# CuzImSlymi/Apertis-LLM

Measured on NVIDIA B200. Metric: SSM+MoE block fwd+bwd tokens/sec, higher is better.
Workload: dtype bf16

## Files before the change

### apertis_llm_b200/_lib.py

```python
from __future__ import annotations

import ctypes
import os
import subprocess
import threading
from ctypes import c_char_p, c_float, c_int, c_int64, c_size_t, c_uint32, c_void_p

import torch

_HERE = os.path.dirname(os.path.abspath(__file__))
LIB_PATH = os.path.join(_HERE, "libapertis_b200.so")
CSRC = os.path.join(_HERE, "csrc")

AB_F32, AB_BF16 = 0, 1
ACT = {"gelu": 0, "relu": 1, "silu": 2, "swish": 2}
EPI_NONE, EPI_BIAS, EPI_BIAS_ACT, EPI_DACT, EPI_ADD = 0, 1, 2, 3, 4
SCAN_SINGLE_PASS, SCAN_TWO_PASS, SCAN_PIPELINED, SCAN_ROUNDS = 0, 1, 2, 3
ROW_ALIGN = 256
ROUTER_EXACT, ROUTER_BF16, ROUTER_FP16 = 0, 1, 2

P, I, I64, SZ, F, U32 = c_void_p, c_int, c_int64, c_size_t, c_float, c_uint32

SIGNATURES = {
    "ab_version": (I, []),
    "ab_device_check": (I, [I]),
    "ab_last_error": (I, [c_char_p, SZ]),
    "ab_causal_conv1d_silu_fwd": (I, [P, I64, P, P, P, I, I, I, I, I, P]),
    "ab_causal_conv1d_silu_bwd_workspace_bytes": (SZ, [I, I, I]),
    "ab_causal_conv1d_silu_bwd": (I, [P, I64, P, P, P, P, I64, P, P, P, SZ, I, I, I, I, I, P]),
    "ab_selective_scan_plan": (I, [I, I, I, I, P, P, P, P, P]),
    "ab_selective_scan_fwd": (I, [P, P, P, P, I64, P, I64, P, P, P, P, P, P, P, P, SZ, U32, I, I, I, I, I, I, P]),
    "ab_selective_scan_bwd": (I, [P, P, P, P, I64, P, I64, P, P, P, P, P, P, P, P, I64, P, P, P, P, P, SZ, U32, I,
                                  I, I, I, I, I, P]),
    "ab_ssm_scan_plan": (I, [I, I, I, I, P, P]),
    "ab_ssm_scan_tune": (I, [I, I, I, I, I]),
    "ab_ssm_scan_fwd": (I, [P, I64, P, I64, P, P, P, I64, P, I64, P, P, P, P, P, P, P, P, SZ, I, I, I, I, I, P]),
    "ab_ssm_scan_bwd": (I, [P, I64, P, P, I64, P, I64, P, P, P, P, P, P, I64, P, P, I64, P, I64, P, I64, I, P, P, P, P, SZ,
                            I, I, I, I, I, P]),
    "ab_gemm_row_tile": (I, []),
    "ab_shifted_ce_fwd": (I, [P, P, P, P, P, P, I, I, I, I64, I, P]),
    "ab_shifted_ce_bwd": (I, [P, P, P, P, P, I, I, I, I64, I, P]),
    "ab_ep_permute_ln": (I, [P, P, P, P, P, P, P, P, I, I, I64, I, I, I64, I, I, P]),
    "ab_ep_unpermute_bwd": (I, [P, P, P, P, P, P, P, I, I, I64, P, F, P, I, I, I64, I, I, I, P]),
    "ab_ep_grouped_gemm_nt": (I, [P, P, P, P, P, I, I, I64, P, P, I64, I, I, I, I, I, I, P]),
    "ab_ep_grouped_gemm_nn": (I, [P, P, P, P, P, I, I, I64, P, P, I64, I, I, I, I, I, I, P]),
    "ab_moe_router_workspace_bytes": (SZ, [I, I, I]),
    "ab_moe_router_fwd": (I, [P, P, P, F, P, P, P, P, P, P, P, P, P, P, P, P, P, P, SZ, I, I, I, I, I, I, P]),
    "ab_moe_topk_from_logits": (I, [P, P, P, P, P, P, I, I, I, P]),
    "ab_moe_max_rows": (I64, [I, I, I, I, I]),
    "ab_moe_plan_workspace_bytes": (SZ, [I, I, I]),
    "ab_moe_plan": (I, [P, P, P, I, P, P, P, P, P, P, P, P, SZ, I, I, I, I, I64, I, P]),
    "ab_moe_permute_ln": (I, [P, P, P, P, P, P, P, P, I, I, I64, I, I, P]),
    "ab_moe_unpermute": (I, [P, P, P, P, P, F, P, I, I, I, I, I, P]),
    "ab_moe_unpermute_bwd": (I, [P, P, P, P, P, P, P, P, F, P, I, I, I64, I, I, I, P]),
    "ab_moe_permute_ln_bwd_workspace_bytes": (SZ, [I, I, I64]),
    "ab_moe_permute_ln_bwd": (I, [P, P, P, P, P, P, P, P, P, P, P, SZ, I, I, I, I64, I, I, P]),
    "ab_moe_segment_colsum_workspace_bytes": (SZ, [I, I, I64]),
    "ab_moe_segment_colsum": (I, [P, P, P, P, P, SZ, I, I, I, I64, I, P]),
    "ab_moe_router_bwd_workspace_bytes": (SZ, [I, I, I]),
    "ab_moe_router_bwd": (I, [P] * 24 + [SZ, I, I, I, I, I, P]),
    "ab_grouped_gemm_nt": (I, [P, P, P, P, P, P, P, P, I64, I, I, I, I, I, I, F, P, P]),
    "ab_grouped_gemm_nn": (I, [P, P, P, P, P, P, P, P, I64, I, I, I, I, I, I, F, P, P]),
    "ab_grouped_gemm_tn_workspace_bytes": (SZ, [I, I, I, I]),
    "ab_grouped_gemm_tn": (I, [P, P, P, P, I64, I, I, I, I, I64, P, SZ, P]),
    "ab_dense_gemm_nt": (I, [P, P, P, P, P, I64, I, I, I, I, P]),
    "ab_dense_gemm_nn": (I, [P, P, P, P, P, I64, I, I, I, I, P]),
    "ab_dense_gemm_tn_workspace_bytes": (SZ, [I64, I, I]),
    "ab_dense_gemm_tn": (I, [P, P, P, P, SZ, I64, I, I, P]),
    "ab_dt_compose_fwd": (I, [P, P, P, I, I, I, I, I, P]),
    "ab_dt_compose_bwd": (I, [P, P, P, P, P, I, I, I, I, P]),
    "ab_layernorm_fwd": (I, [P, P, P, F, P, P, I, I, I, I, P]),
    "ab_layernorm_bwd_workspace_bytes": (SZ, [I, I]),
    "ab_layernorm_bwd": (I, [P, P, P, P, P, P, P, P, P, SZ, I, I, I, I, P]),
    "ab_dropout_add": (I, [P, P, P, F, P, I64, I, I, P]),
    "ab_cast_f32_to_bf16": (I, [P, P, I64, P]),
    "ab_split_f32_to_bf16x3": (I, [P, P, I64, I64, I, P]),
    "ab_split_f32_to_bf16x3_rows": (I, [P, P, P, I, I64, I64, I, P]),
}

_lib = None
_lock = threading.Lock()
_checked_devices = set()


def build(verbose: bool = False) -> str:
    cmd = ["make", "-C", CSRC, "-j", "8"]
    res = subprocess.run(cmd, capture_output=True, text=True)
    if res.returncode != 0:
        raise RuntimeError("building libapertis_b200.so failed:\n" + res.stdout[-4000:] + res.stderr[-4000:])
    if verbose:
        print(res.stdout[-2000:])
    return LIB_PATH


def load() -> ctypes.CDLL:
    global _lib
    with _lock:
        if _lib is not None:
            return _lib
        if not os.path.exists(LIB_PATH):
            build()
        lib = ctypes.CDLL(LIB_PATH)
        for name, (res, args) in SIGNATURES.items():
            fn = getattr(lib, name)
            fn.restype = res
            fn.argtypes = args
        _lib = lib
        return lib


def last_error() -> str:
    buf = ctypes.create_string_buffer(600)
    load().ab_last_error(buf, 600)
    return buf.value.decode("utf-8", "replace")


def ptr(t):
    if t is None:
        return None
    return t.data_ptr()


def dt(t_or_dtype) -> int:
    d = t_or_dtype.dtype if torch.is_tensor(t_or_dtype) else t_or_dtype
    if d == torch.float32:
        return AB_F32
    if d == torch.bfloat16:
        return AB_BF16
    raise TypeError(f"apertis_b200 kernels take float32 or bfloat16 activations, got {d}")


def stream_ptr(device=None) -> int:
    return torch.cuda.current_stream(device).cuda_stream


def ensure_device(device) -> None:
    if device.type != "cuda":
        raise RuntimeError("apertis_llm_b200: the hot path only runs on a CUDA sm_100a (B200) device; got "
                           f"device '{device}'. There is no CPU fallback.")
    idx = device.index if device.index is not None else torch.cuda.current_device()
    if idx in _checked_devices:
        return
    rc = load().ab_device_check(idx)
    if rc != 0:
        raise RuntimeError("apertis_llm_b200: " + last_error())
    _checked_devices.add(idx)


KERNELS_PER_CALL = {
    "ab_causal_conv1d_silu_fwd": 1, "ab_causal_conv1d_silu_bwd": 2,
    "ab_selective_scan_fwd": 1, "ab_selective_scan_bwd": 2,
    "ab_ssm_scan_fwd": 1, "ab_ssm_scan_bwd": 2, "ab_dense_gemm_nt": 1, "ab_dense_gemm_nn": 1, "ab_dense_gemm_tn": 2,
    "ab_dt_compose_fwd": 1, "ab_dt_compose_bwd": 2,
    "ab_moe_router_fwd": 2, "ab_moe_topk_from_logits": 1, "ab_moe_plan": 2, "ab_moe_permute_ln": 1, "ab_moe_unpermute": 1,
    "ab_moe_unpermute_bwd": 1, "ab_moe_permute_ln_bwd": 2, "ab_moe_segment_colsum": 2, "ab_moe_router_bwd": 3,
    "ab_layernorm_fwd": 1, "ab_layernorm_bwd": 3,
    "ab_grouped_gemm_nt": 1, "ab_grouped_gemm_nn": 1, "ab_grouped_gemm_tn": 1, "ab_cast_f32_to_bf16": 1,
    "ab_shifted_ce_fwd": 2, "ab_shifted_ce_bwd": 1, "ab_ep_permute_ln": 1, "ab_ep_unpermute_bwd": 1, "ab_ep_grouped_gemm_nt": 1, "ab_ep_grouped_gemm_nn": 1,
    "ab_split_f32_to_bf16x3": 1, "ab_split_f32_to_bf16x3_rows": 1,
}
launch_count = 0
_timed = None


def start_timing(names):
    global _timed
    _timed = {"names": set(names), "events": []}


def stop_timing():
    global _timed
    t, _timed = _timed, None
    out = {}
    if t is None:
        return out
    torch.cuda.synchronize()
    for name, a, b in t["events"]:
        out.setdefault(name, []).append(a.elapsed_time(b))
    return out


def call(name: str, *args):
    global launch_count
    fn = getattr(load(), name)
    if _timed is not None and name in _timed["names"]:
        a, b = torch.cuda.Event(enable_timing=True), torch.cuda.Event(enable_timing=True)
        a.record()
        rc = fn(*args)
        b.record()
        _timed["events"].append((name, a, b))
    else:
        rc = fn(*args)
    if rc != 0:
        raise RuntimeError(f"{name} failed (code {rc}): {last_error()}")
    launch_count += KERNELS_PER_CALL.get(name, 1)


def query(name: str, *args):
    return getattr(load(), name)(*args)
```

### apertis_llm_b200/csrc/moe_plan.cu

```cuda
#include "common.cuh"

namespace {

template <typename T>
__device__ __forceinline__ void ld4g(const T* p, float* f) {
    if constexpr (sizeof(T) == 4) {
        const float4 q = __ldg(reinterpret_cast<const float4*>(p));
        f[0] = q.x; f[1] = q.y; f[2] = q.z; f[3] = q.w;
    } else {
        const uint2 r = __ldg(reinterpret_cast<const uint2*>(p));
        f[0] = __uint_as_float(r.x << 16); f[1] = __uint_as_float(r.x & 0xffff0000u);
        f[2] = __uint_as_float(r.y << 16); f[3] = __uint_as_float(r.y & 0xffff0000u);
    }
}

constexpr int AB_MAX_PEERS = 16;
struct PeerRows {
    unsigned char* base[AB_MAX_PEERS];
    int n, rows_per_peer, rank;
};
__device__ __forceinline__ unsigned char* peer_row(const PeerRows& pr, void* local, int64_t r, int Dm, int es) {
    if (pr.n == 0) return reinterpret_cast<unsigned char*>(local) + (size_t)r * Dm * es;
    const int d = (int)(r / pr.rows_per_peer);
    const int64_t j = r - (int64_t)d * pr.rows_per_peer;
    return pr.base[d] + ((size_t)pr.rank * pr.rows_per_peer + j) * Dm * es;
}

template <typename T>
__device__ __forceinline__ void st4(T* p, float a, float b, float c, float d) {
    if constexpr (sizeof(T) == 4) {
        *reinterpret_cast<float4*>(p) = make_float4(a, b, c, d);
    } else {
        __nv_bfloat162 lo = __floats2bfloat162_rn(a, b), hi = __floats2bfloat162_rn(c, d);
        *reinterpret_cast<uint2*>(p) = make_uint2(*reinterpret_cast<uint32_t*>(&lo), *reinterpret_cast<uint32_t*>(&hi));
    }
}

constexpr int PLAN_THREADS = 1024;

__device__ __forceinline__ int block_excl_scan(int cnt, int* warp_tot , int& total) {
    const int lane = threadIdx.x & 31, warp = threadIdx.x >> 5;
    int inc = cnt;
#pragma unroll
    for (int o = 1; o < 32; o <<= 1) {
        const int v = __shfl_up_sync(0xffffffffu, inc, o);
        if (lane >= o) inc += v;
    }
    if (lane == 31) warp_tot[warp] = inc;
    __syncthreads();
    int before = 0, tot = 0;
    const int nw = blockDim.x >> 5;
    for (int i = 0; i < nw; ++i) {
        const int c = warp_tot[i];
        if (i < warp) before += c;
        tot += c;
    }
    __syncthreads();
    total = tot;
    return before + inc - cnt;
}

constexpr int TPT = 8;

__device__ __forceinline__ void radix_select_bin(int* hist, int& need, int& sel_bin, int* s_sel_bin, int* s_need) {
    if (threadIdx.x < 32) {
        const int lane = threadIdx.x;
        int h[8], mine = 0;
#pragma unroll
        for (int i = 0; i < 8; ++i) { h[i] = hist[lane * 8 + i]; mine += h[i]; }
        int incl = mine;
#pragma unroll
        for (int o = 1; o < 32; o <<= 1) {
            const int v = __shfl_down_sync(0xffffffffu, incl, o);
            if (lane + o < 32) incl += v;
        }
        const int above = incl - mine;
        const int nd0 = need;
        const bool here = above < nd0 && above + mine >= nd0;
        const unsigned who = __ballot_sync(0xffffffffu, here);
        if (who == 0u) {
            if (lane == 0) { *s_sel_bin = 0; *s_need = nd0 - (above + mine) + h[0]; }
        } else if (lane == __ffs(who) - 1) {
            int nd = nd0 - above, bin = 7;
            for (; bin > 0; --bin) {
                if (h[bin] >= nd) break;
                nd -= h[bin];
            }
            *s_sel_bin = lane * 8 + bin;
            *s_need = nd;
        }
    }
    __syncthreads();
    sel_bin = *s_sel_bin;
    need = *s_need;
    __syncthreads();
}

__device__ __forceinline__ void hist_add_warp(int* hist, bool valid, int bin) {
    const unsigned act = __ballot_sync(0xffffffffu, valid);
    if (valid) {
        const unsigned peers = __match_any_sync(act, bin);
        if ((__ffs(peers) - 1) == (int)(threadIdx.x & 31)) atomicAdd(&hist[bin], __popc(peers));
    }
}

__global__ void __launch_bounds__(PLAN_THREADS) plan_count_kernel(const int32_t* __restrict__ idx, const float* __restrict__ w,
                                                                  const int32_t* __restrict__ active, int cap,
                                                                  int32_t* __restrict__ counts, int32_t* __restrict__ row_local,
                                                                  int S, int K, int list_cap) {
    extern __shared__ uint2 s_list[];
    __shared__ int hist[256];
    __shared__ int warp_tot[32];
    __shared__ int s_sel_bin, s_need;
    const int e = blockIdx.x;
    const int tid = threadIdx.x;
    const bool is_active = active == nullptr || active[e] != 0;
    int kept_total = 0;
    for (int k = 0; k < K; ++k) {
        int n_cand = 0;
        const int span = blockDim.x * TPT;
        for (int s0 = 0; s0 < S; s0 += span) {
            const int sb = s0 + tid * TPT;
            uint32_t wb[TPT];
            bool c[TPT];
            int mine = 0;
#pragma unroll
            for (int t = 0; t < TPT; ++t) {
                const int s = sb + t;
                c[t] = s < S && idx[(size_t)s * K + k] == e;
                wb[t] = c[t] ? __float_as_uint(w[(size_t)s * K + k]) : 0u;
                mine += c[t];
            }
            int tot;
            int pos = n_cand + block_excl_scan(mine, warp_tot, tot);
#pragma unroll
            for (int t = 0; t < TPT; ++t) {
                if (c[t]) {
                    if (pos < list_cap) s_list[pos] = make_uint2((uint32_t)(sb + t), wb[t]);
                    ++pos;
                }
            }
            n_cand += tot;
        }
        __syncthreads();
        const bool in_smem = n_cand <= list_cap;
        const int rem = cap - kept_total;
        int mode = 0;
        if (is_active && n_cand > 0 && rem > 0) mode = n_cand <= rem ? 1 : 2;
        uint32_t tau = 0;
        int n_eq_take = 0;
        if (mode == 2) {
            uint32_t prefix = 0, mask = 0;
            int need = rem, bin;
            for (int pass = 3; pass >= 0; --pass) {
                for (int i = tid; i < 256; i += blockDim.x) hist[i] = 0;
                __syncthreads();
                if (in_smem) {
                    for (int i0 = 0; i0 < n_cand; i0 += blockDim.x) {
                        const int i = i0 + tid;
                        const uint32_t b = i < n_cand ? s_list[i].y : 0u;
                        hist_add_warp(hist, i < n_cand && (b & mask) == prefix, (int)((b >> (8 * pass)) & 0xff));
                    }
                } else {
                    for (int s0 = 0; s0 < S; s0 += blockDim.x) {
                        const int s = s0 + tid;
                        const bool c = s < S && idx[(size_t)s * K + k] == e;
                        const uint32_t b = c ? __float_as_uint(w[(size_t)s * K + k]) : 0u;
                        hist_add_warp(hist, c && (b & mask) == prefix, (int)((b >> (8 * pass)) & 0xff));
                    }
                }
                __syncthreads();
                radix_select_bin(hist, need, bin, &s_sel_bin, &s_need);
                prefix |= (uint32_t)bin << (8 * pass);
                mask |= 0xffu << (8 * pass);
            }
            tau = prefix;
            n_eq_take = need;
        }
        int run_eq = 0, run_kept = 0;
        const int n_items = in_smem ? n_cand : S;
        for (int s0 = 0; s0 < n_items; s0 += span) {
            const int ib = s0 + tid * TPT;
            bool c[TPT], gt[TPT], eq[TPT];
            int tokv[TPT];
            int n_eq = 0;
#pragma unroll
            for (int t = 0; t < TPT; ++t) {
                const int i = ib + t;
                uint32_t b = 0u;
                if (in_smem) {
                    c[t] = i < n_cand;
                    if (c[t]) { const uint2 it = s_list[i]; tokv[t] = (int)it.x; b = it.y; } else tokv[t] = 0;
                } else {
                    c[t] = i < S && idx[(size_t)i * K + k] == e;
                    tokv[t] = i;
                    if (c[t]) b = __float_as_uint(w[(size_t)i * K + k]);
                }
                gt[t] = c[t] && (mode == 1 || (mode == 2 && b > tau));
                eq[t] = c[t] && mode == 2 && b == tau;
                n_eq += eq[t];
            }
            int tot_eq = 0, tot_kept = 0;
            int eq_rank = run_eq;
            if (mode == 2) eq_rank += block_excl_scan(n_eq, warp_tot, tot_eq);
            bool kept[TPT];
            int n_kept = 0;
#pragma unroll
            for (int t = 0; t < TPT; ++t) {
                kept[t] = gt[t] || (eq[t] && eq_rank < n_eq_take);
                eq_rank += eq[t];
                n_kept += kept[t];
            }
            int pos = kept_total + run_kept + block_excl_scan(n_kept, warp_tot, tot_kept);
#pragma unroll
            for (int t = 0; t < TPT; ++t) {
                if (c[t]) row_local[(size_t)tokv[t] * K + k] = kept[t] ? pos : -1;
                pos += kept[t];
            }
            run_eq += tot_eq;
            run_kept += tot_kept;
        }
        kept_total += run_kept;
        __syncthreads();
    }
    if (tid == 0) counts[e] = kept_total;
}

__global__ void plan_finalize_kernel(const int32_t* __restrict__ idx, const int32_t* __restrict__ counts,
                                     const int32_t* __restrict__ row_local, int32_t* __restrict__ seg_off,
                                     int32_t* __restrict__ row_of, int32_t* __restrict__ tok_of_row,
                                     int32_t* __restrict__ slot_of_row, int32_t* __restrict__ tile_expert,
                                     int32_t* __restrict__ n_rows, int S, int K, int E, int align, int64_t max_rows,
                                     int fixed_seg) {
    __shared__ int soff[34];
    if (threadIdx.x == 0) {
        int o = 0, kept = 0;
        for (int e = 0; e < E; ++e) {
            soff[e] = o;
            if (fixed_seg > 0 && counts[e] > fixed_seg) __trap();
            o += fixed_seg > 0 ? fixed_seg : (counts[e] + align - 1) / align * align;
            kept += counts[e];
        }
        soff[E] = o;
        soff[E + 1] = kept;
    }
    __syncthreads();
    if (blockIdx.x == 0) {
        for (int i = threadIdx.x; i <= E; i += blockDim.x) seg_off[i] = soff[i];
        if (threadIdx.x == 0) { n_rows[0] = soff[E]; n_rows[1] = soff[E + 1]; }
        const int ntiles = (int)(max_rows / align);
        for (int t = threadIdx.x; t < ntiles; t += blockDim.x) {
            const int r = t * align;
            int ex = -1;
            for (int e = 0; e < E; ++e)
                if (r >= soff[e] && r < soff[e + 1]) ex = e;
            tile_expert[t] = ex;
        }
    }
    const int64_t n = (int64_t)S * K;
    for (int64_t i = (int64_t)blockIdx.x * blockDim.x + threadIdx.x; i < n; i += (int64_t)gridDim.x * blockDim.x) {
        const int rl = row_local[i];
        if (rl >= 0) {
            const int r = soff[idx[i]] + rl;
            row_of[i] = r;
            tok_of_row[r] = (int)(i / K);
            slot_of_row[r] = (int)(i % K);
        } else {
            row_of[i] = -1;
        }
    }
}

template <typename TI, typename TO>
__global__ void __launch_bounds__(256) permute_ln_kernel(const TI* __restrict__ x, const float* __restrict__ stats,
                                                         const float* __restrict__ ln_w, const float* __restrict__ ln_b,
                                                         const int32_t* __restrict__ tok_of_row,
                                                         const int32_t* __restrict__ tile_expert,
                                                         const int32_t* __restrict__ n_rows, TO* __restrict__ xn, int Dm,
                                                         int align, const PeerRows pr) {
    const int lane = threadIdx.x & 31;
    const int wpb = blockDim.x >> 5;
    const int total = n_rows[0];
    for (int r = blockIdx.x * wpb + (threadIdx.x >> 5); r < total; r += gridDim.x * wpb) {
        const int tok = tok_of_row[r];
        TO* orow = reinterpret_cast<TO*>(peer_row(pr, xn, r, Dm, (int)sizeof(TO)));
        if (tok < 0) {
            for (int d = lane * 4; d < Dm; d += 128) st4<TO>(orow + d, 0.f, 0.f, 0.f, 0.f);
            continue;
        }
        const int e = tile_expert[r / align];
        const float mean = stats[2 * (size_t)tok], rstd = stats[2 * (size_t)tok + 1];
        const TI* irow = x + (size_t)tok * Dm;
        const float* g = ln_w + (size_t)e * Dm;
        const float* bb = ln_b + (size_t)e * Dm;
        for (int d = lane * 4; d < Dm; d += 128) {
            const float4 gv = __ldg(reinterpret_cast<const float4*>(g + d));
            const float4 bv = __ldg(reinterpret_cast<const float4*>(bb + d));
            float xv[4];
#pragma unroll
            for (int v = 0; v < 4; ++v) xv[v] = ab_to_float(irow[d + v]);
            const float o0 = fmaf((xv[0] - mean) * rstd, gv.x, bv.x), o1 = fmaf((xv[1] - mean) * rstd, gv.y, bv.y);
            const float o2 = fmaf((xv[2] - mean) * rstd, gv.z, bv.z), o3 = fmaf((xv[3] - mean) * rstd, gv.w, bv.w);
            st4<TO>(orow + d, o0, o1, o2, o3);
        }
    }
}

template <typename TY, typename TO, int KM>
__global__ void __launch_bounds__(256) unpermute_kernel(const TY* __restrict__ y, const int32_t* __restrict__ row_of,
                                                        const float* __restrict__ w, const float* __restrict__ res, TO* __restrict__ out,
                                                        const uint32_t* __restrict__ seed, uint32_t thresh, float scale, int S, int K, int Dm) {
    constexpr int DU = 8 / KM;
    const int lane = threadIdx.x & 31;
    const int wpb = blockDim.x >> 5;
    uint32_t s0 = 0, s1 = 0;
    if (seed) { s0 = __ldg(seed); s1 = __ldg(seed + 1); }
    for (int s = blockIdx.x * wpb + (threadIdx.x >> 5); s < S; s += gridDim.x * wpb) {
        TO* orow = out + (size_t)s * Dm;
        const TY* rows[KM];
        float wk[KM];
        int rid[KM];
#pragma unroll
        for (int k = 0; k < KM; ++k) {
            rid[k] = k < K ? row_of[(size_t)s * K + k] : -1;
            wk[k] = rid[k] >= 0 ? w[(size_t)s * K + k] : 0.f;
            rows[k] = rid[k] >= 0 ? y + (size_t)rid[k] * Dm : nullptr;
        }
        for (int d0 = lane * 4; d0 < Dm; d0 += 128 * DU) {
            float yv[DU][KM][4];
#pragma unroll
            for (int u = 0; u < DU; ++u) {
                const int d = d0 + u * 128;
#pragma unroll
                for (int k = 0; k < KM; ++k) {
                    if (k < K && rows[k] != nullptr && d < Dm) ld4g<TY>(rows[k] + d, yv[u][k]);
                    else { yv[u][k][0] = yv[u][k][1] = yv[u][k][2] = yv[u][k][3] = 0.f; }
                }
            }
#pragma unroll
            for (int u = 0; u < DU; ++u) {
                const int d = d0 + u * 128;
                if (d >= Dm) break;
                float acc[4] = {0.f, 0.f, 0.f, 0.f};
#pragma unroll
                for (int k = 0; k < KM; ++k) {
                    if (k < K && rows[k] != nullptr) {
#pragma unroll
                        for (int v = 0; v < 4; ++v) acc[v] += yv[u][k][v] * wk[k];
                    }
                }
                if (seed) {
#pragma unroll
                    for (int v = 0; v < 4; ++v) acc[v] = ab_out_keep(s0, s1, (uint64_t)s * Dm + d + v, thresh) ? acc[v] * scale : 0.f;
                }
                if (res) {
                    const float4 rr = *reinterpret_cast<const float4*>(res + (size_t)s * Dm + d);
                    acc[0] += rr.x; acc[1] += rr.y; acc[2] += rr.z; acc[3] += rr.w;
                }
                st4<TO>(orow + d, acc[0], acc[1], acc[2], acc[3]);
            }
        }
    }
}

template <typename TD, typename TY, typename TO>
__global__ void __launch_bounds__(256) unpermute_bwd_kernel(const TD* __restrict__ dout, const TY* __restrict__ y,
                                                            const float* __restrict__ w, const int32_t* __restrict__ tok_of_row,
                                                            const int32_t* __restrict__ slot_of_row,
                                                            const int32_t* __restrict__ n_rows, TO* __restrict__ dy,
                                                            float* __restrict__ dw_row, const uint32_t* __restrict__ seed, uint32_t thresh,
                                                            float scale, int K, int Dm, const PeerRows pr) {
    const int lane = threadIdx.x & 31;
    const int wpb = blockDim.x >> 5;
    const int total = n_rows[0];
    uint32_t s0 = 0, s1 = 0;
    if (seed) { s0 = __ldg(seed); s1 = __ldg(seed + 1); }
    for (int r = blockIdx.x * wpb + (threadIdx.x >> 5); r < total; r += gridDim.x * wpb) {
        const int tok = tok_of_row[r];
        TO* orow = reinterpret_cast<TO*>(peer_row(pr, dy, r, Dm, (int)sizeof(TO)));
        if (tok < 0) {
            for (int d = lane * 4; d < Dm; d += 128) st4<TO>(orow + d, 0.f, 0.f, 0.f, 0.f);
            if (lane == 0) dw_row[r] = 0.f;
            continue;
        }
        const float wk = w[(size_t)tok * K + slot_of_row[r]];
        const TD* drow = dout + (size_t)tok * Dm;
        const TY* yrow = y + (size_t)r * Dm;
        float dot = 0.f;
        for (int d = lane * 4; d < Dm; d += 128) {
            float o[4];
#pragma unroll
            for (int v = 0; v < 4; ++v) {
                float g = ab_to_float(drow[d + v]);
                if (seed) g = ab_out_keep(s0, s1, (uint64_t)tok * Dm + d + v, thresh) ? g * scale : 0.f;
                dot = fmaf(g, ab_to_float(yrow[d + v]), dot);
                o[v] = g * wk;
            }
            st4<TO>(orow + d, o[0], o[1], o[2], o[3]);
        }
        dot = ab_warp_sum(dot);
        if (lane == 0) dw_row[r] = dot;
    }
}

template <typename TX, typename TG>
__global__ void __launch_bounds__(256) permute_ln_bwd_rows_kernel(const TG* __restrict__ dxn, const TX* __restrict__ x,
                                                                  const float* __restrict__ stats, const float* __restrict__ ln_w,
                                                                  const int32_t* __restrict__ tok_of_row,
                                                                  const int32_t* __restrict__ tile_expert,
                                                                  const int32_t* __restrict__ n_rows, float* __restrict__ dxrow,
                                                                  int Dm, int align) {
    const int lane = threadIdx.x & 31, wpb = blockDim.x >> 5;
    const int total = n_rows[0];
    for (int r = blockIdx.x * wpb + (threadIdx.x >> 5); r < total; r += gridDim.x * wpb) {
        const int tok = tok_of_row[r];
        if (tok < 0) continue;
        const int e = tile_expert[r / align];
        const float* g = ln_w + (size_t)e * Dm;
        const float mean = stats[2 * (size_t)tok], rstd = stats[2 * (size_t)tok + 1];
        const TX* xr = x + (size_t)tok * Dm;
        const TG* gr = dxn + (size_t)r * Dm;
        float a1 = 0.f, a2 = 0.f;
        for (int d = lane * 4; d < Dm; d += 128) {
            const float4 gv = __ldg(reinterpret_cast<const float4*>(g + d));
            const float gg[4] = {gv.x, gv.y, gv.z, gv.w};
#pragma unroll
            for (int v = 0; v < 4; ++v) {
                const float dh = ab_to_float(gr[d + v]) * gg[v];
                const float xh = (ab_to_float(xr[d + v]) - mean) * rstd;
                a1 += dh;
                a2 = fmaf(dh, xh, a2);
            }
        }
        const float m1 = ab_warp_sum(a1) / (float)Dm, m2 = ab_warp_sum(a2) / (float)Dm;
        float* orow = dxrow + (size_t)r * Dm;
        for (int d = lane * 4; d < Dm; d += 128) {
            const float4 gv = __ldg(reinterpret_cast<const float4*>(g + d));
            const float gg[4] = {gv.x, gv.y, gv.z, gv.w};
            float o[4];
#pragma unroll
            for (int v = 0; v < 4; ++v) {
                const float dh = ab_to_float(gr[d + v]) * gg[v];
                const float xh = (ab_to_float(xr[d + v]) - mean) * rstd;
                o[v] = rstd * (dh - m1 - xh * m2);
            }
            *reinterpret_cast<float4*>(orow + d) = make_float4(o[0], o[1], o[2], o[3]);
        }
    }
}

template <typename TX, typename TG, int NIT>
__global__ void __launch_bounds__(256, NIT <= 6 ? 3 : 2) permute_ln_bwd_fused_kernel(const TG* __restrict__ dxn, const TX* __restrict__ x,
                                                                   const float* __restrict__ stats, const float* __restrict__ ln_w,
                                                                   const int32_t* __restrict__ tok_of_row,
                                                                   const int32_t* __restrict__ tile_expert,
                                                                   const int32_t* __restrict__ n_rows, float* __restrict__ dxrow,
                                                                   float* __restrict__ part, int Dm, int align, int ratio) {
    __shared__ float sacc[2][NIT * 128];
    const int t = blockIdx.x;
    if ((int64_t)t * align >= n_rows[0]) return;
    const int e = tile_expert[t / ratio];
    if (e < 0) return;
    const int lane = threadIdx.x & 31, warp = threadIdx.x >> 5, wpb = blockDim.x >> 5;
    const float* g = ln_w + (size_t)e * Dm;
    float gw[NIT][4], gb[NIT][4];
#pragma unroll
    for (int it = 0; it < NIT; ++it) {
#pragma unroll
        for (int v = 0; v < 4; ++v) { gw[it][v] = 0.f; gb[it][v] = 0.f; }
    }
    int tok_cur = tok_of_row[t * align + warp];
    int tok_nxt = warp + wpb < align ? tok_of_row[t * align + warp + wpb] : -1;
    for (int i = warp; i < align; i += wpb) {
        const int r = t * align + i;
        const int tok = tok_cur;
        tok_cur = tok_nxt;
        tok_nxt = i + 2 * wpb < align ? tok_of_row[t * align + i + 2 * wpb] : -1;
        if (tok_cur >= 0) {
            const char* px = reinterpret_cast<const char*>(x + (size_t)tok_cur * Dm);
            const char* pg = reinterpret_cast<const char*>(dxn + (size_t)(r + wpb) * Dm);
            for (int o = lane * 128; o < Dm * (int)sizeof(TX); o += 32 * 128) asm volatile("prefetch.global.L1 [%0];" ::"l"(px + o));
            for (int o = lane * 128; o < Dm * (int)sizeof(TG); o += 32 * 128) asm volatile("prefetch.global.L1 [%0];" ::"l"(pg + o));
        }
        if (tok < 0) continue;
        const float mean = stats[2 * (size_t)tok], rstd = stats[2 * (size_t)tok + 1];
        const TX* xr = x + (size_t)tok * Dm;
        const TG* gr = dxn + (size_t)r * Dm;
        float a1 = 0.f, a2 = 0.f;
#pragma unroll
        for (int it = 0; it < NIT; ++it) {
            const int d = it * 128 + lane * 4;
            if (d < Dm) {
                float fx[4], fg[4], gg[4];
                ld4g<TX>(xr + d, fx);
                ld4g<TG>(gr + d, fg);
                ld4g<float>(g + d, gg);
#pragma unroll
                for (int v = 0; v < 4; ++v) {
                    const float xh = (fx[v] - mean) * rstd;
                    gw[it][v] = fmaf(fg[v], xh, gw[it][v]);
                    gb[it][v] += fg[v];
                    const float dh = fg[v] * gg[v];
                    a1 += dh;
                    a2 = fmaf(dh, xh, a2);
                }
            }
        }
        const float m1 = ab_warp_sum(a1) / (float)Dm, m2 = ab_warp_sum(a2) / (float)Dm;
        float* orow = dxrow + (size_t)r * Dm;
#pragma unroll
        for (int it = 0; it < NIT; ++it) {
            const int d = it * 128 + lane * 4;
            if (d < Dm) {
                float fx[4], fg[4], gg[4], o[4];
                ld4g<TX>(xr + d, fx);
                ld4g<TG>(gr + d, fg);
                ld4g<float>(g + d, gg);
#pragma unroll
                for (int v = 0; v < 4; ++v) o[v] = rstd * (fg[v] * gg[v] - m1 - (fx[v] - mean) * rstd * m2);
                *reinterpret_cast<float4*>(orow + d) = make_float4(o[0], o[1], o[2], o[3]);
            }
        }
    }
    for (int wv = 0; wv < wpb; ++wv) {
        if (warp == wv) {
#pragma unroll
            for (int it = 0; it < NIT; ++it) {
#pragma unroll
                for (int v = 0; v < 4; ++v) {
                    const int i = it * 128 + lane * 4 + v;
                    sacc[0][i] = wv ? sacc[0][i] + gw[it][v] : gw[it][v];
                    sacc[1][i] = wv ? sacc[1][i] + gb[it][v] : gb[it][v];
                }
            }
        }
        __syncthreads();
    }
    for (int i = threadIdx.x; i < 2 * Dm; i += blockDim.x) {
        const int q = i / Dm, d = i % Dm;
        part[((size_t)t * 2 + q) * Dm + d] = sacc[q][d];
    }
}

template <typename TX, typename TG>
__global__ void __launch_bounds__(256) permute_ln_bwd_cols_kernel(const TG* __restrict__ dxn, const TX* __restrict__ x,
                                                                  const float* __restrict__ stats,
                                                                  const int32_t* __restrict__ tok_of_row,
                                                                  const int32_t* __restrict__ tile_expert,
                                                                  const int32_t* __restrict__ n_rows, float* __restrict__ part,
                                                                  int Dm, int align, int ratio) {
    __shared__ float red[8][2][128];
    const int t = blockIdx.x;
    if ((int64_t)t * align >= n_rows[0] || tile_expert[t / ratio] < 0) return;
    const int lane = threadIdx.x & 31, warp = threadIdx.x >> 5;
    const int d = blockIdx.y * 128 + lane * 4;
    float gw[4] = {0.f, 0.f, 0.f, 0.f}, gb[4] = {0.f, 0.f, 0.f, 0.f};
    if (d < Dm) {
        for (int i = warp; i < align; i += 8) {
            const int r = t * align + i;
            const int tok = tok_of_row[r];
            if (tok < 0) continue;
            const float mean = stats[2 * (size_t)tok], rstd = stats[2 * (size_t)tok + 1];
#pragma unroll
            for (int v = 0; v < 4; ++v) {
                const float dv = ab_to_float(dxn[(size_t)r * Dm + d + v]);
                const float xh = (ab_to_float(x[(size_t)tok * Dm + d + v]) - mean) * rstd;
                gw[v] = fmaf(dv, xh, gw[v]);
                gb[v] += dv;
            }
        }
    }
#pragma unroll
    for (int v = 0; v < 4; ++v) { red[warp][0][lane * 4 + v] = gw[v]; red[warp][1][lane * 4 + v] = gb[v]; }
    __syncthreads();
    const int q = threadIdx.x >> 7, c = threadIdx.x & 127;
    float s2 = 0.f;
#pragma unroll
    for (int wv = 0; wv < 8; ++wv) s2 += red[wv][q][c];
    const int dd = blockIdx.y * 128 + c;
    if (dd < Dm) part[((size_t)t * 2 + q) * Dm + dd] = s2;
}

template <typename T>
__global__ void __launch_bounds__(256) tile_colsum_kernel(const T* __restrict__ a, const int32_t* __restrict__ tile_expert,
                                                          const int32_t* __restrict__ n_rows, float* __restrict__ part, int C,
                                                          int align, int ratio) {
    __shared__ float red[8][256];
    const int t = blockIdx.x;
    if ((int64_t)t * align >= n_rows[0] || tile_expert[t / ratio] < 0) return;
    const int lane = threadIdx.x & 31, warp = threadIdx.x >> 5;
    const int c0 = blockIdx.y * 256 + lane * 8;
    float acc[8];
#pragma unroll
    for (int v = 0; v < 8; ++v) acc[v] = 0.f;
    if (c0 < C) {
        constexpr int VN = 16 / (int)sizeof(T);
        for (int i0 = warp; i0 < align; i0 += 32) {
            uint4 q[4][8 / VN];
#pragma unroll
            for (int u = 0; u < 4; ++u) {
                const int i = i0 + u * 8;
                const uint4* row = reinterpret_cast<const uint4*>(a + ((size_t)t * align + i) * C + c0);
#pragma unroll
                for (int w = 0; w < 8 / VN; ++w) q[u][w] = i < align ? __ldg(row + w) : make_uint4(0u, 0u, 0u, 0u);
            }
#pragma unroll
            for (int u = 0; u < 4; ++u) {
#pragma unroll
                for (int w = 0; w < 8 / VN; ++w) {
                    float f[VN];
                    ab_vec16<T>::unpack(q[u][w], f);
#pragma unroll
                    for (int v = 0; v < VN; ++v) acc[w * VN + v] += f[v];
                }
            }
        }
    }
#pragma unroll
    for (int v = 0; v < 8; ++v) red[warp][lane * 8 + v] = acc[v];
    __syncthreads();
    const int c = threadIdx.x;
    float s2 = 0.f;
#pragma unroll
    for (int wv = 0; wv < 8; ++wv) s2 += red[wv][c];
    if (blockIdx.y * 256 + c < C) part[(size_t)t * C + blockIdx.y * 256 + c] = s2;
}

__global__ void tile_reduce_kernel(const float* __restrict__ part, const int32_t* __restrict__ tile_expert,
                                   const int32_t* __restrict__ n_rows, float* __restrict__ out_a, float* __restrict__ out_b,
                                   int split, int ncols, int align, int ratio) {
    __shared__ int s_t0, s_t1;
    __shared__ int s_list[1024];
    __shared__ int s_n;
    const int e = blockIdx.y;
    const int ntiles = n_rows[0] / align;
    if (threadIdx.x < 32) {
        int n = 0, t0 = ntiles, t1 = 0;
        for (int base = 0; base < ntiles; base += 32) {
            const int t = base + (int)threadIdx.x;
            const bool mine = t < ntiles && tile_expert[t / ratio] == e;
            const unsigned m = __ballot_sync(0xffffffffu, mine);
            if (mine) {
                const int pos = n + __popc(m & ((1u << threadIdx.x) - 1u));
                if (pos < 1024) s_list[pos] = t;
            }
            if (m) { t0 = min(t0, base + __ffs(m) - 1); t1 = base + 32 - __clz(m); }
            n += __popc(m);
        }
        if (threadIdx.x == 0) { s_t0 = t0; s_t1 = t1; s_n = n; }
    }
    __syncthreads();
    const int j = blockIdx.x * blockDim.x + threadIdx.x;
    if (j >= ncols) return;
    float s = 0.f;
    if (s_n <= 1024) {
        for (int i0 = 0; i0 < s_n; i0 += 8) {
            float v[8];
#pragma unroll
            for (int u = 0; u < 8; ++u) v[u] = i0 + u < s_n ? part[(size_t)s_list[i0 + u] * ncols + j] : 0.f;
#pragma unroll
            for (int u = 0; u < 8; ++u) s += v[u];
        }
    } else {
        for (int t = s_t0; t < s_t1; ++t)
            if (tile_expert[t / ratio] == e) s += part[(size_t)t * ncols + j];
    }
    if (j < split) out_a[(size_t)e * split + j] = s;
    else out_b[(size_t)e * (ncols - split) + (j - split)] = s;
}

int work_rows(int row_align) { return row_align % 128 == 0 ? 128 : row_align; }

int make_peers(PeerRows* pr, const uint64_t* peer_ptrs, int W, int rank, int64_t rows_per_peer) {
    memset(pr, 0, sizeof(*pr));
    if (peer_ptrs == nullptr) return AB_OK;
    AB_REQUIRE(W >= 1 && W <= AB_MAX_PEERS && rank >= 0 && rank < W && rows_per_peer > 0 && rows_per_peer < (1ll << 31),
               "ep: bad peer table (W=%d, rank=%d, rows_per_peer=%lld; at most %d ranks)", W, rank, (long long)rows_per_peer, AB_MAX_PEERS);
    for (int i = 0; i < W; ++i) {
        AB_REQUIRE(peer_ptrs[i] != 0 && peer_ptrs[i] % 16 == 0, "ep: peer buffer %d is null or not 16-byte aligned", i);
        pr->base[i] = reinterpret_cast<unsigned char*>(peer_ptrs[i]);
    }
    pr->n = W; pr->rows_per_peer = (int)rows_per_peer; pr->rank = rank;
    return AB_OK;
}

int rows_grid(int64_t max_rows) {
    const int64_t want = ab_ceil_div(max_rows, 8);
    const int64_t cap = (int64_t)ab_num_sms() * 8;
    return (int)(want < cap ? want : cap);
}

}

extern "C" int64_t ab_moe_max_rows(int S, int K, int E, int cap, int row_align) {
    int64_t kept = (int64_t)S * K;
    if ((int64_t)E * cap < kept) kept = (int64_t)E * cap;
    return ab_round_up(kept + (int64_t)E * (row_align - 1), row_align);
}

extern "C" size_t ab_moe_plan_workspace_bytes(int S, int K, int E) {
    (void)E;
    return (size_t)ab_round_up((int64_t)S * K * sizeof(int32_t), 256);
}

extern "C" int ab_moe_plan(const int32_t* idx, const float* w, const int32_t* active, int cap, int32_t* counts,
                           int32_t* seg_off, int32_t* row_of, int32_t* tok_of_row, int32_t* slot_of_row,
                           int32_t* tile_expert, int32_t* n_rows, void* ws, size_t ws_bytes, int S, int K, int E,
                           int row_align, int64_t max_rows, int fixed_seg, cudaStream_t stream) {
    AB_REQUIRE(S > 0 && K >= 1 && E >= 1 && E <= 32, "moe_plan: bad shape S=%d K=%d E=%d", S, K, E);
    if (fixed_seg > 0) {
        AB_REQUIRE(fixed_seg % row_align == 0 && (cap >= S || fixed_seg >= cap) && max_rows == (int64_t)E * fixed_seg,
                   "moe_plan: fixed_seg (%d) must be a multiple of %d, >= cap, and max_rows == E*fixed_seg", fixed_seg, row_align);
    } else {
        AB_REQUIRE(row_align > 0 && max_rows % row_align == 0 && max_rows >= ab_moe_max_rows(S, K, E, cap < S ? cap : S, row_align),
                   "moe_plan: max_rows %lld too small or not a multiple of %d", (long long)max_rows, row_align);
    }
    AB_REQUIRE(ws && ws_bytes >= ab_moe_plan_workspace_bytes(S, K, E), "moe_plan: workspace too small");
    int32_t* row_local = (int32_t*)ws;
    AB_CHECK_CUDA(cudaMemsetAsync(tok_of_row, 0xFF, (size_t)max_rows * sizeof(int32_t), stream));
    AB_CHECK_CUDA(cudaMemsetAsync(slot_of_row, 0xFF, (size_t)max_rows * sizeof(int32_t), stream));
    int list_cap = (200 * 1024) / 8;
    if (list_cap > S) list_cap = S;
    const size_t plan_smem = (size_t)list_cap * sizeof(uint2);
    AB_CHECK_CUDA(cudaFuncSetAttribute(plan_count_kernel, cudaFuncAttributeMaxDynamicSharedMemorySize, (int)plan_smem));
    plan_count_kernel<<<E, PLAN_THREADS, plan_smem, stream>>>(idx, w, active, cap, counts, row_local, S, K, list_cap);
    AB_LAUNCH_CHECK();
    const int64_t want = ab_ceil_div((int64_t)S * K, 256);
    const int grid = (int)(want < ab_num_sms() * 4 ? want : ab_num_sms() * 4);
    plan_finalize_kernel<<<grid, 256, 0, stream>>>(idx, counts, row_local, seg_off, row_of, tok_of_row, slot_of_row, tile_expert,
                                                   n_rows, S, K, E, row_align, max_rows, fixed_seg);
    AB_LAUNCH_CHECK();
    return AB_OK;
}

namespace {
int permute_ln_impl(const void* x, const float* stats, const float* ln_w, const float* ln_b, const int32_t* tok_of_row,
                    const int32_t* tile_expert, const int32_t* n_rows, void* xn, int Dm, int row_align, int64_t max_rows, int dtype,
                    int out_dtype, const PeerRows& pr, cudaStream_t stream) {
    AB_REQUIRE(Dm > 0 && Dm % 4 == 0, "moe_permute_ln: hidden size must be a multiple of 4");
    const int grid = rows_grid(max_rows);
#define AB_PLN(TI, TO) permute_ln_kernel<TI, TO><<<grid, 256, 0, stream>>>((const TI*)x, stats, ln_w, ln_b, tok_of_row, tile_expert, n_rows, (TO*)xn, Dm, row_align, pr)
    if (dtype == AB_F32 && out_dtype == AB_F32) AB_PLN(float, float);
    else if (dtype == AB_F32 && out_dtype == AB_BF16) AB_PLN(float, __nv_bfloat16);
    else if (dtype == AB_BF16 && out_dtype == AB_BF16) AB_PLN(__nv_bfloat16, __nv_bfloat16);
    else if (dtype == AB_BF16 && out_dtype == AB_F32) AB_PLN(__nv_bfloat16, float);
    else AB_REQUIRE(false, "moe_permute_ln: bad dtypes");
#undef AB_PLN
    AB_LAUNCH_CHECK();
    return AB_OK;
}
}

extern "C" int ab_moe_permute_ln(const void* x, const float* stats, const float* ln_w, const float* ln_b,
                                 const int32_t* tok_of_row, const int32_t* tile_expert, const int32_t* n_rows, void* xn, int Dm,
                                 int row_align, int64_t max_rows, int dtype, int out_dtype, cudaStream_t stream) {
    PeerRows pr;
    make_peers(&pr, nullptr, 0, 0, 0);
    return permute_ln_impl(x, stats, ln_w, ln_b, tok_of_row, tile_expert, n_rows, xn, Dm, row_align, max_rows, dtype, out_dtype, pr, stream);
}

extern "C" int ab_ep_permute_ln(const void* x, const float* stats, const float* ln_w, const float* ln_b,
                                const int32_t* tok_of_row, const int32_t* tile_expert, const int32_t* n_rows,
                                const uint64_t* peer_xn, int W, int rank, int64_t rows_per_peer, int Dm, int row_align,
                                int64_t max_rows, int dtype, int out_dtype, cudaStream_t stream) {
    AB_REQUIRE(peer_xn != nullptr && max_rows == (int64_t)W * rows_per_peer, "ep_permute_ln: max_rows must equal W * rows_per_peer");
    PeerRows pr;
    if (int e = make_peers(&pr, peer_xn, W, rank, rows_per_peer)) return e;
    return permute_ln_impl(x, stats, ln_w, ln_b, tok_of_row, tile_expert, n_rows, nullptr, Dm, row_align, max_rows, dtype, out_dtype, pr, stream);
}

extern "C" int ab_moe_unpermute(const void* y, const int32_t* row_of, const float* w, const float* res, void* out, float drop_p,
                                const uint32_t* drop_seed, int S, int K, int Dm, int y_dtype, int out_dtype, cudaStream_t stream) {
    AB_REQUIRE(Dm > 0 && Dm % 4 == 0, "moe_unpermute: hidden size must be a multiple of 4");
    AB_REQUIRE(drop_p >= 0.f && drop_p < 1.f && (drop_p == 0.f || drop_seed), "moe_unpermute: dropout p must be in [0,1) and needs a seed when > 0");
    AB_REQUIRE(res == nullptr || ((uintptr_t)res % 16) == 0, "moe_unpermute: the residual must be 16-byte aligned fp32");
    const uint32_t thresh = (uint32_t)((double)drop_p * 4294967296.0);
    const float scale = drop_p > 0.f ? 1.0f / (1.0f - drop_p) : 1.0f;
    const uint32_t* sd = drop_p > 0.f ? drop_seed : nullptr;
    const int grid = rows_grid(S);
#define AB_UNP(TY, TO)                                                                                                          \
    {                                                                                                                            \
        if (K <= 2) unpermute_kernel<TY, TO, 2><<<grid, 256, 0, stream>>>((const TY*)y, row_of, w, res, (TO*)out, sd, thresh, scale, S, K, Dm); \
        else if (K <= 4) unpermute_kernel<TY, TO, 4><<<grid, 256, 0, stream>>>((const TY*)y, row_of, w, res, (TO*)out, sd, thresh, scale, S, K, Dm); \
        else unpermute_kernel<TY, TO, 8><<<grid, 256, 0, stream>>>((const TY*)y, row_of, w, res, (TO*)out, sd, thresh, scale, S, K, Dm); \
    }
    AB_REQUIRE(K >= 1 && K <= 8, "moe_unpermute: experts_per_token must be in [1, 8]");
    if (y_dtype == AB_F32 && out_dtype == AB_F32) AB_UNP(float, float)
    else if (y_dtype == AB_BF16 && out_dtype == AB_F32) AB_UNP(__nv_bfloat16, float)
    else if (y_dtype == AB_BF16 && out_dtype == AB_BF16) AB_UNP(__nv_bfloat16, __nv_bfloat16)
    else if (y_dtype == AB_F32 && out_dtype == AB_BF16) AB_UNP(float, __nv_bfloat16)
    else AB_REQUIRE(false, "moe_unpermute: bad dtypes");
#undef AB_UNP
    AB_LAUNCH_CHECK();
    return AB_OK;
}

namespace {
int unpermute_bwd_impl(const void* dout, const void* y, const float* w, const int32_t* tok_of_row, const int32_t* slot_of_row,
                       const int32_t* n_rows, void* dy, float* dw_row, float drop_p, const uint32_t* drop_seed, int K, int Dm,
                       int64_t max_rows, int dout_dtype, int y_dtype, int dy_dtype, const PeerRows& pr, cudaStream_t stream) {
    AB_REQUIRE(Dm > 0 && Dm % 4 == 0, "moe_unpermute_bwd: hidden size must be a multiple of 4");
    AB_REQUIRE(drop_p >= 0.f && drop_p < 1.f && (drop_p == 0.f || drop_seed), "moe_unpermute_bwd: dropout p must be in [0,1) and needs a seed when > 0");
    const uint32_t thresh = (uint32_t)((double)drop_p * 4294967296.0);
    const float scale = drop_p > 0.f ? 1.0f / (1.0f - drop_p) : 1.0f;
    const uint32_t* sd = drop_p > 0.f ? drop_seed : nullptr;
    const int grid = rows_grid(max_rows);
#define AB_UB(TD, TY, TO) unpermute_bwd_kernel<TD, TY, TO><<<grid, 256, 0, stream>>>((const TD*)dout, (const TY*)y, w, tok_of_row, slot_of_row, n_rows, (TO*)dy, dw_row, sd, thresh, scale, K, Dm, pr)
    const int key = dout_dtype * 4 + y_dtype * 2 + dy_dtype;
    switch (key) {
        case 0: AB_UB(float, float, float); break;
        case 1: AB_UB(float, float, __nv_bfloat16); break;
        case 2: AB_UB(float, __nv_bfloat16, float); break;
        case 3: AB_UB(float, __nv_bfloat16, __nv_bfloat16); break;
        case 4: AB_UB(__nv_bfloat16, float, float); break;
        case 5: AB_UB(__nv_bfloat16, float, __nv_bfloat16); break;
        case 6: AB_UB(__nv_bfloat16, __nv_bfloat16, float); break;
        case 7: AB_UB(__nv_bfloat16, __nv_bfloat16, __nv_bfloat16); break;
        default: AB_REQUIRE(false, "moe_unpermute_bwd: bad dtypes");
    }
#undef AB_UB
    AB_LAUNCH_CHECK();
    return AB_OK;
}
}

extern "C" int ab_moe_unpermute_bwd(const void* dout, const void* y, const float* w, const int32_t* tok_of_row,
                                    const int32_t* slot_of_row, const int32_t* n_rows, void* dy, float* dw_row, float drop_p,
                                    const uint32_t* drop_seed, int K, int Dm, int64_t max_rows, int dout_dtype, int y_dtype,
                                    int dy_dtype, cudaStream_t stream) {
    PeerRows pr;
    make_peers(&pr, nullptr, 0, 0, 0);
    return unpermute_bwd_impl(dout, y, w, tok_of_row, slot_of_row, n_rows, dy, dw_row, drop_p, drop_seed, K, Dm, max_rows, dout_dtype,
                              y_dtype, dy_dtype, pr, stream);
}

extern "C" int ab_ep_unpermute_bwd(const void* dout, const void* y, const float* w, const int32_t* tok_of_row,
                                   const int32_t* slot_of_row, const int32_t* n_rows, const uint64_t* peer_dy, int W, int rank,
                                   int64_t rows_per_peer, float* dw_row, float drop_p, const uint32_t* drop_seed, int K, int Dm,
                                   int64_t max_rows, int dout_dtype, int y_dtype, int dy_dtype, cudaStream_t stream) {
    AB_REQUIRE(peer_dy != nullptr && max_rows == (int64_t)W * rows_per_peer, "ep_unpermute_bwd: max_rows must equal W * rows_per_peer");
    PeerRows pr;
    if (int e = make_peers(&pr, peer_dy, W, rank, rows_per_peer)) return e;
    return unpermute_bwd_impl(dout, y, w, tok_of_row, slot_of_row, n_rows, nullptr, dw_row, drop_p, drop_seed, K, Dm, max_rows,
                              dout_dtype, y_dtype, dy_dtype, pr, stream);
}

extern "C" size_t ab_moe_permute_ln_bwd_workspace_bytes(int Dm, int row_align, int64_t max_rows) {
    return (size_t)ab_round_up((max_rows / work_rows(row_align)) * 2 * (int64_t)Dm * sizeof(float), 256);
}

extern "C" int ab_moe_permute_ln_bwd(const void* dxn, const void* x, const float* stats, const float* ln_w,
                                     const int32_t* tok_of_row, const int32_t* tile_expert, const int32_t* n_rows, float* dxrow,
                                     float* dln_w, float* dln_b, void* ws, size_t ws_bytes, int Dm, int E, int row_align,
                                     int64_t max_rows, int dtype, int dxn_dtype, cudaStream_t stream) {
    AB_REQUIRE(ws && ws_bytes >= ab_moe_permute_ln_bwd_workspace_bytes(Dm, row_align, max_rows), "moe_permute_ln_bwd: workspace too small");
    AB_REQUIRE(Dm % 4 == 0, "moe_permute_ln_bwd: hidden size must be a multiple of 4");
    const int sub = work_rows(row_align), ratio = row_align / sub;
    const int ntiles = (int)(max_rows / sub);
    float* part = (float*)ws;
    const int rgrid = rows_grid(max_rows);
    dim3 cgrid(ntiles, (unsigned)ab_ceil_div(Dm, 128));
    const int nit = (int)ab_ceil_div(Dm, 128);
#define AB_LNB_F(TX, TG, NIT)                                                                                                    \
    permute_ln_bwd_fused_kernel<TX, TG, NIT><<<ntiles, 256, 0, stream>>>((const TG*)dxn, (const TX*)x, stats, ln_w, tok_of_row, \
                                                                         tile_expert, n_rows, dxrow, part, Dm, sub, ratio)
#define AB_LNB(TX, TG)                                                                                                           \
    {                                                                                                                            \
        if (nit <= 8) {                                                                                                          \
            if (nit <= 2) AB_LNB_F(TX, TG, 2); else if (nit <= 4) AB_LNB_F(TX, TG, 4);                                           \
            else if (nit <= 6) AB_LNB_F(TX, TG, 6); else AB_LNB_F(TX, TG, 8);                                                    \
        } else {                                                                                                                 \
            permute_ln_bwd_rows_kernel<TX, TG><<<rgrid, 256, 0, stream>>>((const TG*)dxn, (const TX*)x, stats, ln_w, tok_of_row, \
                                                                          tile_expert, n_rows, dxrow, Dm, row_align);            \
            permute_ln_bwd_cols_kernel<TX, TG><<<cgrid, 256, 0, stream>>>((const TG*)dxn, (const TX*)x, stats, tok_of_row,       \
                                                                          tile_expert, n_rows, part, Dm, sub, ratio);            \
        }                                                                                                                        \
    }
    if (dtype == AB_F32 && dxn_dtype == AB_F32) AB_LNB(float, float)
    else if (dtype == AB_F32 && dxn_dtype == AB_BF16) AB_LNB(float, __nv_bfloat16)
    else if (dtype == AB_BF16 && dxn_dtype == AB_BF16) AB_LNB(__nv_bfloat16, __nv_bfloat16)
    else if (dtype == AB_BF16 && dxn_dtype == AB_F32) AB_LNB(__nv_bfloat16, float)
    else AB_REQUIRE(false, "moe_permute_ln_bwd: bad dtypes");
#undef AB_LNB
#undef AB_LNB_F
    AB_LAUNCH_CHECK();
    dim3 grid((unsigned)ab_ceil_div(2 * Dm, 128), E);
    tile_reduce_kernel<<<grid, 128, 0, stream>>>(part, tile_expert, n_rows, dln_w, dln_b, Dm, 2 * Dm, sub, ratio);
    AB_LAUNCH_CHECK();
    return AB_OK;
}

extern "C" size_t ab_moe_segment_colsum_workspace_bytes(int C, int row_align, int64_t max_rows) {
    return (size_t)ab_round_up((max_rows / work_rows(row_align)) * (int64_t)C * sizeof(float), 256);
}

extern "C" int ab_moe_segment_colsum(const void* a, const int32_t* tile_expert, const int32_t* n_rows, float* out, void* ws,
                                     size_t ws_bytes, int C, int E, int row_align, int64_t max_rows, int dtype,
                                     cudaStream_t stream) {
    AB_REQUIRE(ws && ws_bytes >= ab_moe_segment_colsum_workspace_bytes(C, row_align, max_rows), "moe_segment_colsum: workspace too small");
    const int sub = work_rows(row_align), ratio = row_align / sub;
    const int ntiles = (int)(max_rows / sub);
    float* part = (float*)ws;
    AB_REQUIRE(C % 8 == 0 && ((uintptr_t)a % 16) == 0, "moe_segment_colsum: column count must be a multiple of 8 and the matrix 16-byte aligned");
    dim3 cgrid(ntiles, (unsigned)ab_ceil_div(C, 256));
    if (dtype == AB_F32) tile_colsum_kernel<float><<<cgrid, 256, 0, stream>>>((const float*)a, tile_expert, n_rows, part, C, sub, ratio);
    else tile_colsum_kernel<__nv_bfloat16><<<cgrid, 256, 0, stream>>>((const __nv_bfloat16*)a, tile_expert, n_rows, part, C, sub, ratio);
    AB_LAUNCH_CHECK();
    dim3 grid((unsigned)ab_ceil_div(C, 128), E);
    tile_reduce_kernel<<<grid, 128, 0, stream>>>(part, tile_expert, n_rows, out, nullptr, C, C, sub, ratio);
    AB_LAUNCH_CHECK();
    return AB_OK;
}
```

### apertis_llm_b200/csrc/moe_router.cu

```cuda
#include <cuda_fp16.h>

#include "common.cuh"

namespace {

constexpr int WARPS = 8;
constexpr int MAX_K = 8;

__device__ __forceinline__ float ab_round_to(float v, int quant) {
    if (quant == AB_ROUTER_BF16) return __bfloat162float(__float2bfloat16_rn(v));
    if (quant == AB_ROUTER_FP16) return __half2float(__float2half_rn(v));
    return v;
}

template <typename T>
__device__ __forceinline__ void row_load(const T* row, int i, float* f) {
    ab_vec16<T>::unpack(__ldg(reinterpret_cast<const uint4*>(row) + i), f);
}

__device__ __forceinline__ void select_topk(float logit, int lane, int E, int K, float& g, float& lse, int& my_idx, float& my_p,
                                            float& den, unsigned& sel_mask) {
    const float lv = lane < E ? logit : -INFINITY;
    const float m = ab_warp_max(lv);
    const float ex = lane < E ? expf(lv - m) : 0.f;
    const float sum = ab_warp_sum(ex);
    g = ex / sum;
    lse = m + logf(sum);
    float cand = lane < E ? g : -INFINITY;
    my_idx = 0; my_p = 0.f; den = 0.f; sel_mask = 0u;
    for (int k = 0; k < K; ++k) {
        const float best = ab_warp_max(cand);
        const unsigned ball = __ballot_sync(0xffffffffu, cand == best);
        const int win = __ffs(ball) - 1;
        if (lane == k) { my_idx = win; my_p = best; }
        den += best;
        sel_mask |= 1u << win;
        if (lane == win) cand = -INFINITY;
    }
    den += 1e-6f;
}

__device__ __forceinline__ void write_selection(int s, int lane, int E, int K, float g, float lse, int my_idx, float my_p, float den,
                                                float* gates, int32_t* idx, float* probs, float* w, float* lse_out) {
    if (lane < E) gates[(size_t)s * E + lane] = g;
    if (lane < K) {
        idx[(size_t)s * K + lane] = my_idx;
        probs[(size_t)s * K + lane] = my_p;
        w[(size_t)s * K + lane] = my_p / den;
    }
    if (lane == 0) lse_out[s] = lse;
}

template <typename T, int EM>
__global__ void __launch_bounds__(WARPS * 32) router_fwd_kernel(const T* __restrict__ x, const float* __restrict__ ln_w,
                                                                const float* __restrict__ ln_b, float eps,
                                                                const float* __restrict__ Wr, const float* __restrict__ br,
                                                                const float* __restrict__ noise,
                                                                const float* __restrict__ noise_scale, float* __restrict__ lclean,
                                                                float* __restrict__ logits, float* __restrict__ gates,
                                                                int32_t* __restrict__ idx, float* __restrict__ probs,
                                                                float* __restrict__ w, float* __restrict__ lse_out,
                                                                float* __restrict__ stats, float* __restrict__ part, int S,
                                                                int Dm, int E, int K, int quant) {
    constexpr int V = ab_vec16<T>::N;
    extern __shared__ float sm[];
    float* G = sm;
    float* cvec = G + (size_t)E * Dm;
    float* red = cvec + 32;
    float* lnw_s = red + WARPS * (2 * E + 1);
    float* lnb_s = lnw_s + Dm;
    const int tid = threadIdx.x, lane = tid & 31, warp = tid >> 5;
    if (quant == AB_ROUTER_EXACT) {
        for (int e = 0; e < E; ++e)
            for (int d = tid; d < Dm; d += blockDim.x) G[(size_t)e * Dm + d] = ln_w[d] * Wr[(size_t)e * Dm + d];
        for (int e = warp; e < E; e += WARPS) {
            float acc = 0.f;
            for (int d = lane; d < Dm; d += 32) acc = fmaf(ln_b[d], Wr[(size_t)e * Dm + d], acc);
            acc = ab_warp_sum(acc);
            if (lane == 0) cvec[e] = acc + br[e];
        }
    } else {
        for (int e = 0; e < E; ++e)
            for (int d = tid; d < Dm; d += blockDim.x) G[(size_t)e * Dm + d] = ab_round_to(Wr[(size_t)e * Dm + d], quant);
        for (int d = tid; d < Dm; d += blockDim.x) { lnw_s[d] = ln_w[d]; lnb_s[d] = ln_b[d]; }
        if (tid < E) cvec[tid] = ab_round_to(br[tid], quant);
    }
    __syncthreads();
    const int nvec = Dm / V;
    float a_g = 0.f, a_cnt = 0.f, a_l2 = 0.f;
    for (int s = blockIdx.x * WARPS + warp; s < S; s += gridDim.x * WARPS) {
        const T* row = x + (size_t)s * Dm;
        float sum = 0.f;
        for (int i = lane; i < nvec; i += 32) {
            float f[V];
            row_load<T>(row, i, f);
#pragma unroll
            for (int v = 0; v < V; ++v) sum += f[v];
        }
        const float mean = ab_warp_sum(sum) / (float)Dm;
        float var = 0.f;
        float dot[EM];
#pragma unroll
        for (int e = 0; e < EM; ++e) dot[e] = 0.f;
        for (int i = lane; i < nvec; i += 32) {
            float f[V];
            row_load<T>(row, i, f);
#pragma unroll
            for (int v = 0; v < V; ++v) { f[v] -= mean; var = fmaf(f[v], f[v], var); }
#pragma unroll
            for (int e = 0; e < EM; ++e) {
                if (e < E) {
#pragma unroll
                    for (int v4 = 0; v4 < V; v4 += 4) {
                        const float4 gq = *reinterpret_cast<const float4*>(G + (size_t)e * Dm + i * V + v4);
                        dot[e] = fmaf(f[v4], gq.x, dot[e]); dot[e] = fmaf(f[v4 + 1], gq.y, dot[e]);
                        dot[e] = fmaf(f[v4 + 2], gq.z, dot[e]); dot[e] = fmaf(f[v4 + 3], gq.w, dot[e]);
                    }
                }
            }
        }
        var = ab_warp_sum(var) / (float)Dm;
        const float rstd = rsqrtf(var + eps);
        if (quant != AB_ROUTER_EXACT) {
#pragma unroll
            for (int e = 0; e < EM; ++e) dot[e] = 0.f;
            for (int i = lane; i < nvec; i += 32) {
                float f[V];
                row_load<T>(row, i, f);
#pragma unroll
                for (int v = 0; v < V; ++v) f[v] = ab_round_to(fmaf((f[v] - mean) * rstd, lnw_s[i * V + v], lnb_s[i * V + v]), quant);
#pragma unroll
                for (int e = 0; e < EM; ++e) {
                    if (e < E) {
#pragma unroll
                        for (int v = 0; v < V; ++v) dot[e] = fmaf(f[v], G[(size_t)e * Dm + i * V + v], dot[e]);
                    }
                }
            }
        }
        float mylogit = 0.f;
#pragma unroll
        for (int e = 0; e < EM; ++e) {
            if (e < E) {
                const float t = ab_warp_sum(dot[e]);
                if (lane == e) mylogit = t;
            }
        }
        float lc = 0.f;
        if (lane < E) {
            lc = quant == AB_ROUTER_EXACT ? fmaf(rstd, mylogit, cvec[lane]) : ab_round_to(mylogit + cvec[lane], quant);
            mylogit = lc;
            if (noise) mylogit = fmaf(noise[(size_t)s * E + lane], noise_scale[lane], lc);
            if (lclean) lclean[(size_t)s * E + lane] = lc;
            if (logits) logits[(size_t)s * E + lane] = mylogit;
        }
        if (lane == 0) { stats[2 * (size_t)s] = mean; stats[2 * (size_t)s + 1] = rstd; }
        float g, lse, my_p, den;
        int my_idx;
        unsigned sel_mask;
        select_topk(mylogit, lane, E, K, g, lse, my_idx, my_p, den, sel_mask);
        write_selection(s, lane, E, K, g, lse, my_idx, my_p, den, gates, idx, probs, w, lse_out);
        if (lane < E) {
            a_g += g;
            a_cnt += (sel_mask >> lane) & 1u ? 1.f : 0.f;
        }
        if (lane == 0) a_l2 = fmaf(lse, lse, a_l2);
    }
    const int NA = 2 * E + 1;
    if (lane < E) { red[warp * NA + lane] = a_g; red[warp * NA + E + lane] = a_cnt; }
    if (lane == 0) red[warp * NA + 2 * E] = a_l2;
    __syncthreads();
    if (tid < NA) {
        float s2 = 0.f;
        for (int wv = 0; wv < WARPS; ++wv) s2 += red[wv * NA + tid];
        part[(size_t)blockIdx.x * NA + tid] = s2;
    }
}

template <int EM>
__device__ __forceinline__ float reduce_dots_to_lane(float (&dot)[EM], int lane, int E) {
    float mine = 0.f;
    if (EM == 8) {
        float v4[4], v2[2], v1;
        const bool h16 = lane & 16, h8 = lane & 8, h4 = lane & 4;
#pragma unroll
        for (int j = 0; j < 4; ++j) {
            const float keep = h16 ? dot[4 + j] : dot[j], send = h16 ? dot[j] : dot[4 + j];
            v4[j] = keep + __shfl_xor_sync(0xffffffffu, send, 16);
        }
#pragma unroll
        for (int j = 0; j < 2; ++j) {
            const float keep = h8 ? v4[2 + j] : v4[j], send = h8 ? v4[j] : v4[2 + j];
            v2[j] = keep + __shfl_xor_sync(0xffffffffu, send, 8);
        }
        {
            const float keep = h4 ? v2[1] : v2[0], send = h4 ? v2[0] : v2[1];
            v1 = keep + __shfl_xor_sync(0xffffffffu, send, 4);
        }
        v1 += __shfl_xor_sync(0xffffffffu, v1, 2);
        v1 += __shfl_xor_sync(0xffffffffu, v1, 1);
        const int src = ((lane >> 2) & 1) << 4 | ((lane >> 1) & 1) << 3 | (lane & 1) << 2;
        mine = __shfl_sync(0xffffffffu, v1, src);
        if (lane >= E) mine = 0.f;
    } else {
#pragma unroll
        for (int e = 0; e < EM; ++e) {
            if (e < E) {
                const float t = ab_warp_sum(dot[e]);
                if (lane == e) mine = t;
            }
        }
    }
    return mine;
}

template <typename T, int EM, int NV>
__global__ void __launch_bounds__(WARPS * 32, (NV * ab_vec16<T>::N <= 24 && EM <= 8) ? 4 : 1) router_fwd_reg_kernel(const T* __restrict__ x, const float* __restrict__ ln_w,
                                                                    const float* __restrict__ ln_b, float eps,
                                                                    const float* __restrict__ Wr, const float* __restrict__ br,
                                                                    const float* __restrict__ noise,
                                                                    const float* __restrict__ noise_scale, float* __restrict__ lclean,
                                                                    float* __restrict__ logits, float* __restrict__ gates,
                                                                    int32_t* __restrict__ idx, float* __restrict__ probs,
                                                                    float* __restrict__ w, float* __restrict__ lse_out,
                                                                    float* __restrict__ stats, float* __restrict__ part, int S,
                                                                    int Dm, int E, int K, int quant) {
    constexpr int V = ab_vec16<T>::N;
    extern __shared__ float sm[];
    float* G = sm;
    float* cvec = G + (size_t)E * Dm;
    float* red = cvec + 32;
    float* lnw_s = red + WARPS * (2 * E + 1);
    float* lnb_s = lnw_s + Dm;
    const int tid = threadIdx.x, lane = tid & 31, warp = tid >> 5;
    if (quant == AB_ROUTER_EXACT) {
        for (int i = tid; i < E * Dm; i += blockDim.x) G[i] = ln_w[i % Dm] * Wr[i];
        for (int e = warp; e < E; e += WARPS) {
            float acc = 0.f;
            for (int d = lane; d < Dm; d += 32) acc = fmaf(ln_b[d], Wr[(size_t)e * Dm + d], acc);
            acc = ab_warp_sum(acc);
            if (lane == 0) cvec[e] = acc + br[e];
        }
    } else {
        for (int i = tid; i < E * Dm; i += blockDim.x) G[i] = ab_round_to(Wr[i], quant);
        for (int d = tid; d < Dm; d += blockDim.x) { lnw_s[d] = ln_w[d]; lnb_s[d] = ln_b[d]; }
        if (tid < E) cvec[tid] = ab_round_to(br[tid], quant);
    }
    __syncthreads();
    const int nvec = Dm / V;
    const float inv_dm = 1.0f / (float)Dm;
    float a_g = 0.f, a_cnt = 0.f, a_l2 = 0.f;
    for (int s = blockIdx.x * WARPS + warp; s < S; s += gridDim.x * WARPS) {
        const T* row = x + (size_t)s * Dm;
        float f[NV][V];
        float sum = 0.f;
#pragma unroll
        for (int i = 0; i < NV; ++i) {
            const int iv = i * 32 + lane;
            if (iv < nvec) {
                row_load<T>(row, iv, f[i]);
#pragma unroll
                for (int v = 0; v < V; ++v) sum += f[i][v];
            } else {
#pragma unroll
                for (int v = 0; v < V; ++v) f[i][v] = 0.f;
            }
        }
        const float mean = ab_warp_sum(sum) * inv_dm;
        float var = 0.f;
#pragma unroll
        for (int i = 0; i < NV; ++i) {
            if (i * 32 + lane < nvec) {
#pragma unroll
                for (int v = 0; v < V; ++v) { f[i][v] -= mean; var = fmaf(f[i][v], f[i][v], var); }
            }
        }
        var = ab_warp_sum(var) * inv_dm;
        const float rstd = rsqrtf(var + eps);
        float dot[EM];
#pragma unroll
        for (int e = 0; e < EM; ++e) dot[e] = 0.f;
#pragma unroll
        for (int i = 0; i < NV; ++i) {
            const int iv = i * 32 + lane;
            if (iv < nvec) {
                if (quant != AB_ROUTER_EXACT) {
#pragma unroll
                    for (int v4 = 0; v4 < V; v4 += 4) {
                        const float4 lw = *reinterpret_cast<const float4*>(lnw_s + iv * V + v4);
                        const float4 lb = *reinterpret_cast<const float4*>(lnb_s + iv * V + v4);
                        f[i][v4] = ab_round_to(fmaf(f[i][v4] * rstd, lw.x, lb.x), quant);
                        f[i][v4 + 1] = ab_round_to(fmaf(f[i][v4 + 1] * rstd, lw.y, lb.y), quant);
                        f[i][v4 + 2] = ab_round_to(fmaf(f[i][v4 + 2] * rstd, lw.z, lb.z), quant);
                        f[i][v4 + 3] = ab_round_to(fmaf(f[i][v4 + 3] * rstd, lw.w, lb.w), quant);
                    }
                }
#pragma unroll
                for (int e = 0; e < EM; ++e) {
                    if (e < E) {
#pragma unroll
                        for (int v4 = 0; v4 < V; v4 += 4) {
                            const float4 gq = *reinterpret_cast<const float4*>(G + (size_t)e * Dm + iv * V + v4);
                            dot[e] = fmaf(f[i][v4], gq.x, dot[e]); dot[e] = fmaf(f[i][v4 + 1], gq.y, dot[e]);
                            dot[e] = fmaf(f[i][v4 + 2], gq.z, dot[e]); dot[e] = fmaf(f[i][v4 + 3], gq.w, dot[e]);
                        }
                    }
                }
            }
        }
        float mylogit = reduce_dots_to_lane<EM>(dot, lane, E);
        float lc = 0.f;
        if (lane < E) {
            lc = quant == AB_ROUTER_EXACT ? fmaf(rstd, mylogit, cvec[lane]) : ab_round_to(mylogit + cvec[lane], quant);
            mylogit = lc;
            if (noise) mylogit = fmaf(noise[(size_t)s * E + lane], noise_scale[lane], lc);
            if (lclean) lclean[(size_t)s * E + lane] = lc;
            if (logits) logits[(size_t)s * E + lane] = mylogit;
        }
        if (lane == 0) { stats[2 * (size_t)s] = mean; stats[2 * (size_t)s + 1] = rstd; }
        float g, lse, my_p, den;
        int my_idx;
        unsigned sel_mask;
        select_topk(mylogit, lane, E, K, g, lse, my_idx, my_p, den, sel_mask);
        write_selection(s, lane, E, K, g, lse, my_idx, my_p, den, gates, idx, probs, w, lse_out);
        if (lane < E) {
            a_g += g;
            a_cnt += (sel_mask >> lane) & 1u ? 1.f : 0.f;
        }
        if (lane == 0) a_l2 = fmaf(lse, lse, a_l2);
    }
    const int NA = 2 * E + 1;
    if (lane < E) { red[warp * NA + lane] = a_g; red[warp * NA + E + lane] = a_cnt; }
    if (lane == 0) red[warp * NA + 2 * E] = a_l2;
    __syncthreads();
    if (tid < NA) {
        float s2 = 0.f;
        for (int wv = 0; wv < WARPS; ++wv) s2 += red[wv * NA + tid];
        part[(size_t)blockIdx.x * NA + tid] = s2;
    }
}

__global__ void reduce_rows_kernel(const float* __restrict__ part, int nrows, int ncols, float* __restrict__ out) {
    const int c = blockIdx.x * (blockDim.x >> 5) + (threadIdx.x >> 5);
    const int lane = threadIdx.x & 31;
    if (c >= ncols) return;
    float s = 0.f;
    for (int r = lane; r < nrows; r += 32) s += part[(size_t)r * ncols + c];
    s = ab_warp_sum(s);
    if (lane == 0) out[c] = s;
}

__global__ void __launch_bounds__(WARPS * 32) topk_from_logits_kernel(const float* __restrict__ logits, float* __restrict__ gates,
                                                                      int32_t* __restrict__ idx, float* __restrict__ probs,
                                                                      float* __restrict__ w, float* __restrict__ lse_out, int S,
                                                                      int E, int K) {
    const int lane = threadIdx.x & 31, warp = threadIdx.x >> 5;
    for (int s = blockIdx.x * WARPS + warp; s < S; s += gridDim.x * WARPS) {
        const float l = lane < E ? logits[(size_t)s * E + lane] : 0.f;
        float g, lse, my_p, den;
        int my_idx;
        unsigned sel_mask;
        select_topk(l, lane, E, K, g, lse, my_idx, my_p, den, sel_mask);
        write_selection(s, lane, E, K, g, lse, my_idx, my_p, den, gates, idx, probs, w, lse_out);
    }
}

template <typename T, int EM>
__global__ void __launch_bounds__(WARPS * 32) router_bwd_kernel(const T* __restrict__ x, const float* __restrict__ stats,
                                                                const float* __restrict__ ln_w, const float* __restrict__ ln_b,
                                                                const float* __restrict__ Wr, const float* __restrict__ br,
                                                                const float* __restrict__ gates, const int32_t* __restrict__ idx,
                                                                const float* __restrict__ probs, const float* __restrict__ lse,
                                                                const float* __restrict__ lclean, const float* __restrict__ noise,
                                                                const float* __restrict__ f, const float* __restrict__ scal,
                                                                const float* __restrict__ dw_row, const float* __restrict__ dxrow,
                                                                const int32_t* __restrict__ row_of, T* __restrict__ dx,
                                                                float* __restrict__ dlogits, float* __restrict__ part, int S,
                                                                int Dm, int E, int K) {
    constexpr int V = ab_vec16<T>::N;
    extern __shared__ float sm[];
    float* Wsm = sm;
    float* gam = Wsm + (size_t)E * Dm;
    float* GS = gam + Dm;
    float* cvec = GS + 32;
    float* red = cvec + 32;
    const int tid = threadIdx.x, lane = tid & 31, warp = tid >> 5;
    for (int i = tid; i < E * Dm; i += blockDim.x) Wsm[i] = Wr[i];
    for (int i = tid; i < Dm; i += blockDim.x) gam[i] = ln_w[i];
    for (int e = warp; e < E; e += WARPS) {
        float a1 = 0.f, a2 = 0.f;
        for (int d = lane; d < Dm; d += 32) {
            a1 = fmaf(ln_w[d], Wr[(size_t)e * Dm + d], a1);
            a2 = fmaf(ln_b[d], Wr[(size_t)e * Dm + d], a2);
        }
        a1 = ab_warp_sum(a1); a2 = ab_warp_sum(a2);
        if (lane == 0) { GS[e] = a1; cvec[e] = a2 + br[e]; }
    }
    __syncthreads();
    const float g_lb = scal[0], g_rz = scal[1];
    const int nvec = Dm / V;
    float a_db = 0.f, a_dn = 0.f;
    for (int s = blockIdx.x * WARPS + warp; s < S; s += gridDim.x * WARPS) {
        int my_r = -1, my_i = 0;
        float my_dw = 0.f, my_pk = 0.f;
        if (lane < K) {
            my_r = row_of[(size_t)s * K + lane];
            my_i = idx[(size_t)s * K + lane];
            my_pk = probs[(size_t)s * K + lane];
            my_dw = my_r >= 0 ? dw_row[my_r] : 0.f;
        }
        float den = 0.f;
        for (int k = 0; k < K; ++k) den += __shfl_sync(0xffffffffu, my_pk, k);
        den += 1e-6f;
        const float dot = ab_warp_sum(my_dw * my_pk);
        const float inv = 1.f / den;
        const float my_dp = my_dw * inv - dot * inv * inv;
        float dgate = 0.f, g = 0.f;
        for (int k = 0; k < K; ++k) {
            const int ik = __shfl_sync(0xffffffffu, my_i, k);
            const float dpk = __shfl_sync(0xffffffffu, my_dp, k);
            if (lane == ik) dgate += dpk;
        }
        if (lane < E) {
            g = gates[(size_t)s * E + lane];
            dgate = fmaf(g_lb, f[lane], dgate);
        } else {
            dgate = 0.f;
        }
        const float gd = ab_warp_sum(g * dgate);
        float dl = 0.f;
        if (lane < E) {
            dl = g * (dgate - gd) + g_rz * 2.f * lse[s] * g;
            dlogits[(size_t)s * E + lane] = dl;
            a_db += dl;
            if (noise) a_dn = fmaf(dl, noise[(size_t)s * E + lane], a_dn);
        }
        const float mean = stats[2 * (size_t)s], rstd = stats[2 * (size_t)s + 1];
        float t1 = 0.f, t2 = 0.f;
        if (lane < E) {
            t1 = dl * GS[lane];
            t2 = dl * (lclean[(size_t)s * E + lane] - cvec[lane]);
        }
        const float m1 = ab_warp_sum(t1) / (float)Dm;
        const float m2 = ab_warp_sum(t2) / (float)Dm;
        float dle[EM];
#pragma unroll
        for (int e = 0; e < EM; ++e) dle[e] = __shfl_sync(0xffffffffu, dl, e);
        int rk[MAX_K];
#pragma unroll
        for (int k = 0; k < MAX_K; ++k) { const int r = __shfl_sync(0xffffffffu, my_r, k); rk[k] = k < K ? r : -1; }
        const T* row = x + (size_t)s * Dm;
        T* orow = dx + (size_t)s * Dm;
        for (int i = lane; i < nvec; i += 32) {
            float fx[V], o[V];
            row_load<T>(row, i, fx);
            float dxn[V];
#pragma unroll
            for (int v = 0; v < V; ++v) dxn[v] = 0.f;
#pragma unroll
            for (int e = 0; e < EM; ++e) {
                if (e < E) {
#pragma unroll
                    for (int v4 = 0; v4 < V; v4 += 4) {
                        const float4 wq = *reinterpret_cast<const float4*>(Wsm + (size_t)e * Dm + i * V + v4);
                        dxn[v4] = fmaf(dle[e], wq.x, dxn[v4]); dxn[v4 + 1] = fmaf(dle[e], wq.y, dxn[v4 + 1]);
                        dxn[v4 + 2] = fmaf(dle[e], wq.z, dxn[v4 + 2]); dxn[v4 + 3] = fmaf(dle[e], wq.w, dxn[v4 + 3]);
                    }
                }
            }
#pragma unroll
            for (int v4 = 0; v4 < V; v4 += 4) {
                const float4 gq = *reinterpret_cast<const float4*>(gam + i * V + v4);
                const float gg[4] = {gq.x, gq.y, gq.z, gq.w};
#pragma unroll
                for (int u = 0; u < 4; ++u) {
                    const float xh = (fx[v4 + u] - mean) * rstd;
                    o[v4 + u] = rstd * (dxn[v4 + u] * gg[u] - m1 - xh * m2);
                }
            }
#pragma unroll
            for (int k = 0; k < MAX_K; ++k) {
                const int rkk = rk[k];
                if (rkk >= 0) {
                    const float* er = dxrow + (size_t)rkk * Dm + i * V;
#pragma unroll
                    for (int v4 = 0; v4 < V; v4 += 4) {
                        const float4 q = __ldg(reinterpret_cast<const float4*>(er + v4));
                        o[v4] += q.x; o[v4 + 1] += q.y; o[v4 + 2] += q.z; o[v4 + 3] += q.w;
                    }
                }
            }
            *(reinterpret_cast<uint4*>(orow) + i) = ab_vec16<T>::pack(o);
        }
    }
    const int NA = 2 * E;
    if (lane < E) { red[warp * NA + lane] = a_db; red[warp * NA + E + lane] = a_dn; }
    __syncthreads();
    if (tid < NA) {
        float s2 = 0.f;
        for (int wv = 0; wv < WARPS; ++wv) s2 += red[wv * NA + tid];
        part[(size_t)blockIdx.x * NA + tid] = s2;
    }
}

constexpr int qb_for(int em) { return 2048 / em; }
int em_for(int E) { return E <= 8 ? 8 : (E <= 16 ? 16 : 32); }
template <typename T, int EM>
__global__ void __launch_bounds__(256) router_q_kernel(const T* __restrict__ x, const float* __restrict__ stats,
                                                       const float* __restrict__ dlogits, float* __restrict__ qpart, int S,
                                                       int Dm, int E) {
    constexpr int QB = qb_for(EM);
    __shared__ float sdl[QB * EM];
    __shared__ float sst[QB * 2];
    const int s0 = blockIdx.y * QB;
    const int ns = min(QB, S - s0);
    for (int i = threadIdx.x; i < ns * E; i += blockDim.x) sdl[i] = dlogits[(size_t)s0 * E + i];
    for (int i = threadIdx.x; i < ns * 2; i += blockDim.x) sst[i] = stats[(size_t)s0 * 2 + i];
    __syncthreads();
    const int d = blockIdx.x * blockDim.x + threadIdx.x;
    if (d >= Dm) return;
    float acc[EM];
#pragma unroll
    for (int e = 0; e < EM; ++e) acc[e] = 0.f;
    for (int j0 = 0; j0 < ns; j0 += 8) {
        float xv[8];
#pragma unroll
        for (int u = 0; u < 8; ++u) xv[u] = j0 + u < ns ? ab_to_float(x[(size_t)(s0 + j0 + u) * Dm + d]) : 0.f;
#pragma unroll
        for (int u = 0; u < 8; ++u) {
            const int j = j0 + u;
            if (j < ns) {
                const float xh = (xv[u] - sst[2 * j]) * sst[2 * j + 1];
#pragma unroll
                for (int e = 0; e < EM; ++e)
                    if (e < E) acc[e] = fmaf(sdl[j * E + e], xh, acc[e]);
            }
        }
    }
#pragma unroll
    for (int e = 0; e < EM; ++e)
        if (e < E) qpart[((size_t)blockIdx.y * E + e) * Dm + d] = acc[e];
}

__global__ void router_param_kernel(const float* __restrict__ qpart, int nqb, const float* __restrict__ part, int nparts,
                                    const float* __restrict__ ln_w, const float* __restrict__ ln_b, const float* __restrict__ Wr,
                                    float* __restrict__ dWr, float* __restrict__ dbr, float* __restrict__ dln_w,
                                    float* __restrict__ dln_b, float* __restrict__ dnoise_scale, int Dm, int E) {
    __shared__ float sdb[64];
    __shared__ float sgw[32][33], sgb[32][33];
    __shared__ float spart[16][64];
    const int tx = threadIdx.x, e = threadIdx.y;
    const int tid = e * 32 + tx;
    const int nthr = 32 * E;
    {
        const int ncol = 2 * E;
        const int ngrp = min(16, nthr / ncol);
        const int col = tid % ncol, grp = tid / ncol;
        if (grp < ngrp) {
            float s = 0.f;
            for (int r0 = grp; r0 < nparts; r0 += ngrp * 4) {
                float v[4];
#pragma unroll
                for (int u = 0; u < 4; ++u) v[u] = r0 + u * ngrp < nparts ? part[(size_t)(r0 + u * ngrp) * ncol + col] : 0.f;
#pragma unroll
                for (int u = 0; u < 4; ++u) s += v[u];
            }
            spart[grp][col] = s;
        }
        __syncthreads();
        if (tid < ncol) {
            float s = 0.f;
            for (int g2 = 0; g2 < ngrp; ++g2) s += spart[g2][tid];
            sdb[tid] = s;
            if (blockIdx.x == 0) {
                if (tid < E) dbr[tid] = s;
                else if (dnoise_scale) dnoise_scale[tid - E] = s;
            }
        }
    }
    __syncthreads();
    const int d = blockIdx.x * 32 + tx;
    float gw = 0.f, gb = 0.f;
    if (d < Dm) {
        float q = 0.f;
        for (int r0 = 0; r0 < nqb; r0 += 8) {
            float qv[8];
#pragma unroll
            for (int u = 0; u < 8; ++u) qv[u] = r0 + u < nqb ? qpart[((size_t)(r0 + u) * E + e) * Dm + d] : 0.f;
#pragma unroll
            for (int u = 0; u < 8; ++u) q += qv[u];
        }
        const float wv = Wr[(size_t)e * Dm + d];
        dWr[(size_t)e * Dm + d] = fmaf(ln_w[d], q, ln_b[d] * sdb[e]);
        gw = wv * q;
        gb = wv * sdb[e];
    }
    sgw[e][tx] = gw;
    sgb[e][tx] = gb;
    __syncthreads();
    if (e == 0 && d < Dm) {
        float a = 0.f, b = 0.f;
        for (int i = 0; i < E; ++i) { a += sgw[i][tx]; b += sgb[i][tx]; }
        dln_w[d] = a;
        dln_b[d] = b;
    }
}

int router_grid(int S) {
    const int want = (int)ab_ceil_div(S, WARPS);
    const int cap = ab_num_sms() * 4;
    return want < cap ? want : cap;
}

struct FwdWs { size_t part_off, total; int grid; };
FwdWs fwd_ws(int S, int E) {
    FwdWs w;
    w.grid = router_grid(S);
    w.part_off = 0;
    w.total = ab_round_up((int64_t)w.grid * (2 * E + 1) * sizeof(float), 256);
    return w;
}
struct BwdWs { size_t part_off, dl_off, q_off, total; int grid, nqb; };
BwdWs bwd_ws(int S, int Dm, int E) {
    BwdWs w;
    w.grid = router_grid(S);
    w.nqb = (int)ab_ceil_div(S, qb_for(em_for(E)));
    size_t o = 0;
    w.part_off = o; o += ab_round_up((int64_t)w.grid * 2 * E * sizeof(float), 256);
    w.dl_off = o; o += ab_round_up((int64_t)S * E * sizeof(float), 256);
    w.q_off = o; o += ab_round_up((int64_t)w.nqb * E * Dm * sizeof(float), 256);
    w.total = o;
    return w;
}

int check_router(int S, int Dm, int E, int K, int dtype) {
    AB_REQUIRE(S > 0 && Dm > 0, "moe_router: empty shape S=%d Dm=%d", S, Dm);
    AB_REQUIRE(E >= 1 && E <= 32, "moe_router: num_experts must be in [1,32] (got %d)", E);
    AB_REQUIRE(K >= 1 && K <= MAX_K && K <= E, "moe_router: experts_per_token must be in [1,%d] and <= E (got %d)", MAX_K, K);
    AB_REQUIRE(dtype == AB_F32 || dtype == AB_BF16, "moe_router: bad dtype %d", dtype);
    const int V = dtype == AB_F32 ? 4 : 8;
    AB_REQUIRE(Dm % V == 0, "moe_router: hidden size %d must be a multiple of %d", Dm, V);
    return AB_OK;
}

}

extern "C" size_t ab_moe_router_workspace_bytes(int S, int Dm, int E) { (void)Dm; return fwd_ws(S, E).total; }

extern "C" int ab_moe_router_fwd(const void* x, const float* ln_w, const float* ln_b, float eps, const float* Wr,
                                 const float* br, const float* noise, const float* noise_scale, float* lclean, float* logits,
                                 float* gates, int32_t* idx, float* probs, float* w, float* lse, float* stats_out, float* aux,
                                 void* ws, size_t ws_bytes, int S, int Dm, int E, int K, int dtype, int quant, cudaStream_t stream) {
    if (int e = check_router(S, Dm, E, K, dtype)) return e;
    const FwdWs wl = fwd_ws(S, E);
    AB_REQUIRE(ws && ws_bytes >= wl.total, "moe_router_fwd: workspace too small");
    AB_REQUIRE(noise == nullptr || noise_scale != nullptr, "moe_router_fwd: noise without noise_scale");
    AB_REQUIRE(quant == AB_ROUTER_EXACT || quant == AB_ROUTER_BF16 || quant == AB_ROUTER_FP16, "moe_router_fwd: bad logit rounding mode %d", quant);
    const size_t smem = ((size_t)E * Dm + 32 + WARPS * (2 * E + 1) + 2 * (size_t)Dm) * sizeof(float);
    float* part = (float*)ws;
    const int V = dtype == AB_F32 ? 4 : 8;
    const int nv = (int)ab_ceil_div(Dm, 32 * V);
#define AB_ROUTER_LAUNCH(KERNEL)                                                                                        \
    {                                                                                                                    \
        auto k = KERNEL;                                                                                                 \
        AB_CHECK_CUDA(cudaFuncSetAttribute(k, cudaFuncAttributeMaxDynamicSharedMemorySize, (int)smem));                 \
        k<<<wl.grid, WARPS * 32, smem, stream>>>((const TT*)x, ln_w, ln_b, eps, Wr, br, noise, noise_scale, lclean,     \
                                                 logits, gates, idx, probs, w, lse, stats_out, part, S, Dm, E, K, quant); \
    }
#define AB_ROUTER_FWD(TT_, EMV)                                                                                         \
    {                                                                                                                    \
        using TT = TT_;                                                                                                  \
        if (nv <= 4) AB_ROUTER_LAUNCH((router_fwd_reg_kernel<TT, EMV, 4>))                                               \
        else if (nv <= 6) AB_ROUTER_LAUNCH((router_fwd_reg_kernel<TT, EMV, 6>))                                          \
        else if (nv <= 8) AB_ROUTER_LAUNCH((router_fwd_reg_kernel<TT, EMV, 8>))                                          \
        else if (nv <= 16 && EMV <= 8) AB_ROUTER_LAUNCH((router_fwd_reg_kernel<TT, EMV, 16>))                            \
        else AB_ROUTER_LAUNCH((router_fwd_kernel<TT, EMV>))                                                              \
    }
    if (dtype == AB_F32) {
        if (E <= 8) AB_ROUTER_FWD(float, 8) else if (E <= 16) AB_ROUTER_FWD(float, 16) else AB_ROUTER_FWD(float, 32)
    } else {
        if (E <= 8) AB_ROUTER_FWD(__nv_bfloat16, 8) else if (E <= 16) AB_ROUTER_FWD(__nv_bfloat16, 16) else AB_ROUTER_FWD(__nv_bfloat16, 32)
    }
#undef AB_ROUTER_LAUNCH
#undef AB_ROUTER_FWD
    AB_LAUNCH_CHECK();
    reduce_rows_kernel<<<(unsigned)ab_ceil_div(2 * E + 1, 4), 128, 0, stream>>>(part, wl.grid, 2 * E + 1, aux);
    AB_LAUNCH_CHECK();
    return AB_OK;
}

extern "C" int ab_moe_topk_from_logits(const float* logits, float* gates, int32_t* idx, float* probs, float* w, float* lse,
                                       int S, int E, int K, cudaStream_t stream) {
    if (int e = check_router(S, 8, E, K, AB_F32)) return e;
    topk_from_logits_kernel<<<router_grid(S), WARPS * 32, 0, stream>>>(logits, gates, idx, probs, w, lse, S, E, K);
    AB_LAUNCH_CHECK();
    return AB_OK;
}

extern "C" size_t ab_moe_router_bwd_workspace_bytes(int S, int Dm, int E) { return bwd_ws(S, Dm, E).total; }

extern "C" int ab_moe_router_bwd(const void* x, const float* stats, const float* ln_w, const float* ln_b, const float* Wr,
                                 const float* br, const float* gates, const int32_t* idx, const float* probs, const float* lse,
                                 const float* lclean, const float* noise, const float* f, const float* scal,
                                 const float* dw_row, const float* dxrow, const int32_t* row_of, void* dx, float* dWr,
                                 float* dbr, float* dln_w, float* dln_b, float* dnoise_scale, void* ws, size_t ws_bytes, int S,
                                 int Dm, int E, int K, int dtype, cudaStream_t stream) {
    if (int e = check_router(S, Dm, E, K, dtype)) return e;
    AB_REQUIRE(Dm % 4 == 0, "moe_router_bwd: hidden size must be a multiple of 4");
    const BwdWs wl = bwd_ws(S, Dm, E);
    AB_REQUIRE(ws && ws_bytes >= wl.total, "moe_router_bwd: workspace too small");
    unsigned char* w8 = (unsigned char*)ws;
    float* part = (float*)(w8 + wl.part_off);
    float* dl = (float*)(w8 + wl.dl_off);
    float* qpart = (float*)(w8 + wl.q_off);
    const size_t smem = ((size_t)E * Dm + Dm + 64 + WARPS * 2 * E) * sizeof(float);
    dim3 qgrid((unsigned)ab_ceil_div(Dm, 256), wl.nqb);
#define AB_ROUTER_BWD(TT, EMV)                                                                                          \
    {                                                                                                                    \
        auto k = router_bwd_kernel<TT, EMV>;                                                                             \
        AB_CHECK_CUDA(cudaFuncSetAttribute(k, cudaFuncAttributeMaxDynamicSharedMemorySize, (int)smem));                 \
        k<<<wl.grid, WARPS * 32, smem, stream>>>((const TT*)x, stats, ln_w, ln_b, Wr, br, gates, idx, probs, lse,       \
                                                 lclean, noise, f, scal, dw_row, dxrow, row_of, (TT*)dx, dl, part, S,   \
                                                 Dm, E, K);                                                              \
        AB_LAUNCH_CHECK();                                                                                               \
        router_q_kernel<TT, EMV><<<qgrid, 256, 0, stream>>>((const TT*)x, stats, dl, qpart, S, Dm, E);                  \
    }
    if (dtype == AB_F32) {
        if (E <= 8) AB_ROUTER_BWD(float, 8) else if (E <= 16) AB_ROUTER_BWD(float, 16) else AB_ROUTER_BWD(float, 32)
    } else {
        if (E <= 8) AB_ROUTER_BWD(__nv_bfloat16, 8) else if (E <= 16) AB_ROUTER_BWD(__nv_bfloat16, 16) else AB_ROUTER_BWD(__nv_bfloat16, 32)
    }
#undef AB_ROUTER_BWD
    AB_LAUNCH_CHECK();
    router_param_kernel<<<(unsigned)ab_ceil_div(Dm, 32), dim3(32, E), 0, stream>>>(qpart, wl.nqb, part, wl.grid, ln_w, ln_b, Wr, dWr,
                                                                                  dbr, dln_w, dln_b, dnoise_scale, Dm, E);
    AB_LAUNCH_CHECK();
    return AB_OK;
}
```

Before: 14.56 million.

## Parallelize MoE plan across token chunks and fuse router bwd kernels

The MoE capacity planning moves from one 1024-thread block per expert to a multi-CTA pipeline. It runs a grid-wide histogram radix select with last-CTA finalization, then per-chunk counts and a position kernel that uses warp match and ballot. The router forward becomes persistent with a grid capped by occupancy, and the router backward gains a fused token kernel plus a column kernel when E and Dm allow. The param kernel also gets a third grid dimension of groups. This trades a few serial launches for more small kernels and global atomics, which adds launch overhead and extra complexity.

Result: faster. 15.03 million (median of 6 runs) (+3.2%).

```diff
diff --git a/apertis_llm_b200/_lib.py b/apertis_llm_b200/_lib.py
--- a/apertis_llm_b200/_lib.py
+++ b/apertis_llm_b200/_lib.py
@@ -152,7 +152,7 @@
     "ab_selective_scan_fwd": 1, "ab_selective_scan_bwd": 2,
     "ab_ssm_scan_fwd": 1, "ab_ssm_scan_bwd": 2, "ab_dense_gemm_nt": 1, "ab_dense_gemm_nn": 1, "ab_dense_gemm_tn": 2,
     "ab_dt_compose_fwd": 1, "ab_dt_compose_bwd": 2,
-    "ab_moe_router_fwd": 2, "ab_moe_topk_from_logits": 1, "ab_moe_plan": 2, "ab_moe_permute_ln": 1, "ab_moe_unpermute": 1,
+    "ab_moe_router_fwd": 2, "ab_moe_topk_from_logits": 1, "ab_moe_plan": 7, "ab_moe_permute_ln": 1, "ab_moe_unpermute": 1,
     "ab_moe_unpermute_bwd": 1, "ab_moe_permute_ln_bwd": 2, "ab_moe_segment_colsum": 2, "ab_moe_router_bwd": 3,
     "ab_layernorm_fwd": 1, "ab_layernorm_bwd": 3,
     "ab_grouped_gemm_nt": 1, "ab_grouped_gemm_nn": 1, "ab_grouped_gemm_tn": 1, "ab_cast_f32_to_bf16": 1,
diff --git a/apertis_llm_b200/csrc/moe_plan.cu b/apertis_llm_b200/csrc/moe_plan.cu
--- a/apertis_llm_b200/csrc/moe_plan.cu
+++ b/apertis_llm_b200/csrc/moe_plan.cu
@@ -36,64 +36,47 @@
     }
 }
 
-constexpr int PLAN_THREADS = 1024;
-
-__device__ __forceinline__ int block_excl_scan(int cnt, int* warp_tot , int& total) {
-    const int lane = threadIdx.x & 31, warp = threadIdx.x >> 5;
-    int inc = cnt;
+constexpr int PLAN_THREADS = 256;
+constexpr int PLAN_CHUNK = PLAN_THREADS;
+constexpr int HIST_TOKENS = PLAN_THREADS;
+
+struct PlanSel {
+    uint32_t prefix;
+    int need;
+    int mode;
+    int base;
+};
+
+__device__ __forceinline__ void warp_select_bin(const int* hist, int lane, int& need, int& sel_bin) {
+    int h[8], mine = 0;
+#pragma unroll
+    for (int i = 0; i < 8; ++i) { h[i] = hist[lane * 8 + i]; mine += h[i]; }
+    int incl = mine;
 #pragma unroll
     for (int o = 1; o < 32; o <<= 1) {
-        const int v = __shfl_up_sync(0xffffffffu, inc, o);
-        if (lane >= o) inc += v;
-    }
-    if (lane == 31) warp_tot[warp] = inc;
-    __syncthreads();
-    int before = 0, tot = 0;
-    const int nw = blockDim.x >> 5;
-    for (int i = 0; i < nw; ++i) {
-        const int c = warp_tot[i];
-        if (i < warp) before += c;
-        tot += c;
-    }
-    __syncthreads();
-    total = tot;
-    return before + inc - cnt;
-}
-
-constexpr int TPT = 8;
-
-__device__ __forceinline__ void radix_select_bin(int* hist, int& need, int& sel_bin, int* s_sel_bin, int* s_need) {
-    if (threadIdx.x < 32) {
-        const int lane = threadIdx.x;
-        int h[8], mine = 0;
-#pragma unroll
-        for (int i = 0; i < 8; ++i) { h[i] = hist[lane * 8 + i]; mine += h[i]; }
-        int incl = mine;
-#pragma unroll
-        for (int o = 1; o < 32; o <<= 1) {
-            const int v = __shfl_down_sync(0xffffffffu, incl, o);
-            if (lane + o < 32) incl += v;
-        }
-        const int above = incl - mine;
-        const int nd0 = need;
-        const bool here = above < nd0 && above + mine >= nd0;
-        const unsigned who = __ballot_sync(0xffffffffu, here);
-        if (who == 0u) {
-            if (lane == 0) { *s_sel_bin = 0; *s_need = nd0 - (above + mine) + h[0]; }
-        } else if (lane == __ffs(who) - 1) {
-            int nd = nd0 - above, bin = 7;
-            for (; bin > 0; --bin) {
-                if (h[bin] >= nd) break;
-                nd -= h[bin];
-            }
-            *s_sel_bin = lane * 8 + bin;
-            *s_need = nd;
-        }
-    }
-    __syncthreads();
-    sel_bin = *s_sel_bin;
-    need = *s_need;
-    __syncthreads();
+        const int v = __shfl_down_sync(0xffffffffu, incl, o);
+        if (lane + o < 32) incl += v;
+    }
+    const int above = incl - mine;
+    const int nd0 = need;
+    const bool here = above < nd0 && above + mine >= nd0;
+    const unsigned who = __ballot_sync(0xffffffffu, here);
+    int bin = 0, nd = 0;
+    if (who == 0u) {
+        nd = __shfl_sync(0xffffffffu, nd0 - (above + mine) + h[0], 0);
+        bin = 0;
+    } else {
+        const int src = __ffs(who) - 1;
+        int b = 7, n2 = nd0 - above;
+        for (; b > 0; --b) {
+            if (h[b] >= n2) break;
+            n2 -= h[b];
+        }
+        bin = __shfl_sync(0xffffffffu, lane * 8 + b, src);
+        nd = __shfl_sync(0xffffffffu, n2, src);
+    }
+    sel_bin = bin;
+    need = nd;
 }
 
 __device__ __forceinline__ void hist_add_warp(int* hist, bool valid, int bin) {
@@ -104,126 +87,168 @@
     }
 }
 
-__global__ void __launch_bounds__(PLAN_THREADS) plan_count_kernel(const int32_t* __restrict__ idx, const float* __restrict__ w,
-                                                                  const int32_t* __restrict__ active, int cap,
-                                                                  int32_t* __restrict__ counts, int32_t* __restrict__ row_local,
-                                                                  int S, int K, int list_cap) {
-    extern __shared__ uint2 s_list[];
-    __shared__ int hist[256];
-    __shared__ int warp_tot[32];
-    __shared__ int s_sel_bin, s_need;
-    const int e = blockIdx.x;
-    const int tid = threadIdx.x;
-    const bool is_active = active == nullptr || active[e] != 0;
-    int kept_total = 0;
-    for (int k = 0; k < K; ++k) {
-        int n_cand = 0;
-        const int span = blockDim.x * TPT;
-        for (int s0 = 0; s0 < S; s0 += span) {
-            const int sb = s0 + tid * TPT;
-            uint32_t wb[TPT];
-            bool c[TPT];
-            int mine = 0;
-#pragma unroll
-            for (int t = 0; t < TPT; ++t) {
-                const int s = sb + t;
-                c[t] = s < S && idx[(size_t)s * K + k] == e;
-                wb[t] = c[t] ? __float_as_uint(w[(size_t)s * K + k]) : 0u;
-                mine += c[t];
-            }
-            int tot;
-            int pos = n_cand + block_excl_scan(mine, warp_tot, tot);
-#pragma unroll
-            for (int t = 0; t < TPT; ++t) {
-                if (c[t]) {
-                    if (pos < list_cap) s_list[pos] = make_uint2((uint32_t)(sb + t), wb[t]);
-                    ++pos;
-                }
-            }
-            n_cand += tot;
-        }
+__device__ __forceinline__ bool last_cta(int* ticket) {
+    __shared__ bool s_last;
+    __threadfence();
+    __syncthreads();
+    if (threadIdx.x == 0) s_last = atomicAdd(ticket, 1) == (int)(gridDim.x * gridDim.y) - 1;
+    __syncthreads();
+    if (s_last) __threadfence();
+    return s_last;
+}
+
+__global__ void __launch_bounds__(PLAN_THREADS) plan_hist_kernel(const int32_t* __restrict__ idx, const float* __restrict__ w,
+                                                                 const int32_t* __restrict__ active, int cap, int pass,
+                                                                 int* __restrict__ ghist, PlanSel* __restrict__ sel,
+                                                                 int* __restrict__ any_select, int* __restrict__ ticket,
+                                                                 int32_t* __restrict__ counts, int S, int K, int E) {
+    __shared__ int hist[32 * 256];
+    if (pass < 3 && *any_select == 0) return;
+    const int k = blockIdx.y, tid = threadIdx.x;
+    for (int i = tid; i < E * 256; i += blockDim.x) hist[i] = 0;
+    __syncthreads();
+    const int shift = 8 * pass;
+    const uint32_t mask = pass == 3 ? 0u : 0xffffffffu << (shift + 8);
+    const int s_end = min(S, (int)(blockIdx.x + 1) * HIST_TOKENS);
+    for (int s0 = blockIdx.x * HIST_TOKENS; s0 < s_end; s0 += blockDim.x) {
+        const int s = s0 + tid;
+        bool c = s < s_end;
+        int e = 0;
+        uint32_t b = 0u;
+        if (c) {
+            e = idx[(size_t)s * K + k];
+            b = __float_as_uint(w[(size_t)s * K + k]);
+            if (pass < 3) {
+                const PlanSel st = sel[e * K + k];
+                c = st.mode == 2 && (b & mask) == st.prefix;
+            }
+        }
+        hist_add_warp(hist, c, e * 256 + (int)((b >> shift) & 0xffu));
+    }
+    __syncthreads();
+    int* gh = ghist + (size_t)k * 256;
+    for (int i = tid; i < E * 256; i += blockDim.x) {
+        const int h = hist[i];
+        if (h) atomicAdd(&gh[(size_t)(i >> 8) * K * 256 + (i & 255)], h);
+    }
+    if (!last_cta(ticket)) return;
+    const int lane = tid & 31, warp = tid >> 5;
+    int any = 0;
+    for (int e = warp; e < E; e += blockDim.x >> 5) {
+        int kept = 0;
+        for (int kk = 0; kk < K; ++kk) {
+            const int* hk = ghist + ((size_t)e * K + kk) * 256;
+            PlanSel st;
+            if (pass == 3) {
+                int n = 0;
+                for (int i = lane; i < 256; i += 32) n += hk[i];
+                n = __reduce_add_sync(0xffffffffu, n);
+                const bool is_active = active == nullptr || active[e] != 0;
+                const int rem = cap - kept;
+                st.mode = 0;
+                if (is_active && n > 0 && rem > 0) st.mode = n <= rem ? 1 : 2;
+                st.base = kept;
+                st.need = rem;
+                st.prefix = 0u;
+                kept += st.mode == 1 ? n : (st.mode == 2 ? rem : 0);
+            } else {
+                st = sel[e * K + kk];
+            }
+            if (st.mode == 2) {
+                int bin;
+                warp_select_bin(hk, lane, st.need, bin);
+                st.prefix |= (uint32_t)bin << shift;
+                any = 1;
+            }
+            if (lane == 0) sel[e * K + kk] = st;
+        }
+        if (pass == 3 && lane == 0) counts[e] = kept;
+    }
+    if (pass == 3) {
+        __shared__ int s_any;
+        if (tid == 0) s_any = 0;
         __syncthreads();
-        const bool in_smem = n_cand <= list_cap;
-        const int rem = cap - kept_total;
-        int mode = 0;
-        if (is_active && n_cand > 0 && rem > 0) mode = n_cand <= rem ? 1 : 2;
-        uint32_t tau = 0;
-        int n_eq_take = 0;
-        if (mode == 2) {
-            uint32_t prefix = 0, mask = 0;
-            int need = rem, bin;
-            for (int pass = 3; pass >= 0; --pass) {
-                for (int i = tid; i < 256; i += blockDim.x) hist[i] = 0;
-                __syncthreads();
-                if (in_smem) {
-                    for (int i0 = 0; i0 < n_cand; i0 += blockDim.x) {
-                        const int i = i0 + tid;
-                        const uint32_t b = i < n_cand ? s_list[i].y : 0u;
-                        hist_add_warp(hist, i < n_cand && (b & mask) == prefix, (int)((b >> (8 * pass)) & 0xff));
-                    }
-                } else {
-                    for (int s0 = 0; s0 < S; s0 += blockDim.x) {
-                        const int s = s0 + tid;
-                        const bool c = s < S && idx[(size_t)s * K + k] == e;
-                        const uint32_t b = c ? __float_as_uint(w[(size_t)s * K + k]) : 0u;
-                        hist_add_warp(hist, c && (b & mask) == prefix, (int)((b >> (8 * pass)) & 0xff));
-                    }
-                }
-                __syncthreads();
-                radix_select_bin(hist, need, bin, &s_sel_bin, &s_need);
-                prefix |= (uint32_t)bin << (8 * pass);
-                mask |= 0xffu << (8 * pass);
-            }
-            tau = prefix;
-            n_eq_take = need;
-        }
-        int run_eq = 0, run_kept = 0;
-        const int n_items = in_smem ? n_cand : S;
-        for (int s0 = 0; s0 < n_items; s0 += span) {
-            const int ib = s0 + tid * TPT;
-            bool c[TPT], gt[TPT], eq[TPT];
-            int tokv[TPT];
-            int n_eq = 0;
-#pragma unroll
-            for (int t = 0; t < TPT; ++t) {
-                const int i = ib + t;
-                uint32_t b = 0u;
-                if (in_smem) {
-                    c[t] = i < n_cand;
-                    if (c[t]) { const uint2 it = s_list[i]; tokv[t] = (int)it.x; b = it.y; } else tokv[t] = 0;
-                } else {
-                    c[t] = i < S && idx[(size_t)i * K + k] == e;
-                    tokv[t] = i;
-                    if (c[t]) b = __float_as_uint(w[(size_t)i * K + k]);
-                }
-                gt[t] = c[t] && (mode == 1 || (mode == 2 && b > tau));
-                eq[t] = c[t] && mode == 2 && b == tau;
-                n_eq += eq[t];
-            }
-            int tot_eq = 0, tot_kept = 0;
-            int eq_rank = run_eq;
-            if (mode == 2) eq_rank += block_excl_scan(n_eq, warp_tot, tot_eq);
-            bool kept[TPT];
-            int n_kept = 0;
-#pragma unroll
-            for (int t = 0; t < TPT; ++t) {
-                kept[t] = gt[t] || (eq[t] && eq_rank < n_eq_take);
-                eq_rank += eq[t];
-                n_kept += kept[t];
-            }
-            int pos = kept_total + run_kept + block_excl_scan(n_kept, warp_tot, tot_kept);
-#pragma unroll
-            for (int t = 0; t < TPT; ++t) {
-                if (c[t]) row_local[(size_t)tokv[t] * K + k] = kept[t] ? pos : -1;
-                pos += kept[t];
-            }
-            run_eq += tot_eq;
-            run_kept += tot_kept;
-        }
-        kept_total += run_kept;
+        if (any && lane == 0) s_any = 1;
         __syncthreads();
-    }
-    if (tid == 0) counts[e] = kept_total;
+        if (tid == 0) *any_select = s_any;
+    }
+}
+
+__device__ __forceinline__ int plan_class(const PlanSel& st, uint32_t b) {
+    if (st.mode == 1) return 0;
+    if (st.mode == 2) return b > st.prefix ? 0 : (b == st.prefix ? 1 : -1);
+    return -1;
+}
+
+__global__ void __launch_bounds__(PLAN_THREADS) plan_chunk_count_kernel(const int32_t* __restrict__ idx, const float* __restrict__ w,
+                                                                        const PlanSel* __restrict__ sel, int* __restrict__ cc,
+                                                                        int S, int K, int E) {
+    __shared__ int cnt[64];
+    const int k = blockIdx.y, tid = threadIdx.x;
+    if (tid < 2 * E) cnt[tid] = 0;
+    __syncthreads();
+    const int s = blockIdx.x * PLAN_CHUNK + tid;
+    int cls = -1, e = 0;
+    if (s < S) {
+        e = idx[(size_t)s * K + k];
+        cls = plan_class(sel[e * K + k], __float_as_uint(w[(size_t)s * K + k]));
+    }
+    hist_add_warp(cnt, cls >= 0, e * 2 + (cls > 0 ? 1 : 0));
+    __syncthreads();
+    if (tid < 2 * E) cc[((size_t)blockIdx.x * K + k) * 2 * E + tid] = cnt[tid];
+}
+
+__global__ void __launch_bounds__(PLAN_THREADS) plan_pos_kernel(const int32_t* __restrict__ idx, const float* __restrict__ w,
+                                                                const PlanSel* __restrict__ sel, const int* __restrict__ cc,
+                                                                int32_t* __restrict__ row_local, int S, int K, int E) {
+    __shared__ int wcnt[PLAN_THREADS / 32][64];
+    __shared__ int sbase[PLAN_THREADS];
+    const int k = blockIdx.y, tid = threadIdx.x, lane = tid & 31, warp = tid >> 5;
+    {
+        const int ncol = 2 * E, ng = PLAN_THREADS / ncol, col = tid % ncol, grp = tid / ncol;
+        int sum = 0;
+        if (grp < ng)
+            for (int c = grp; c < (int)blockIdx.x; c += ng) sum += cc[((size_t)c * K + k) * ncol + col];
+        sbase[tid] = sum;
+    }
+    const int s = blockIdx.x * PLAN_CHUNK + tid;
+    int cls = -1, e = 0;
+    PlanSel st{0u, 0, 0, 0};
+    if (s < S) {
+        e = idx[(size_t)s * K + k];
+        st = sel[e * K + k];
+        cls = plan_class(st, __float_as_uint(w[(size_t)s * K + k]));
+    }
+    const unsigned valid = __ballot_sync(0xffffffffu, s < S);
+    const unsigned same = __match_any_sync(0xffffffffu, s < S ? e : -1) & valid;
+    const unsigned gtm = __ballot_sync(0xffffffffu, cls == 0), eqm = __ballot_sync(0xffffffffu, cls == 1);
+    const unsigned lt = (1u << lane) - 1u;
+    for (int i = tid; i < (PLAN_THREADS / 32) * 64; i += blockDim.x) (&wcnt[0][0])[i] = 0;
+    __syncthreads();
+    if (s < S && (__ffs(same) - 1) == lane) {
+        wcnt[warp][2 * e] = __popc(same & gtm);
+        wcnt[warp][2 * e + 1] = __popc(same & eqm);
+    }
+    __syncthreads();
+    if (tid < 2 * E) {
+        int run = 0;
+        for (int g = 0; g < PLAN_THREADS / (2 * E); ++g) run += sbase[g * 2 * E + tid];
+        for (int wv = 0; wv < PLAN_THREADS / 32; ++wv) {
+            const int v = wcnt[wv][tid];
+            wcnt[wv][tid] = run;
+            run += v;
+        }
+    }
+    __syncthreads();
+    if (s < S) {
+        int r = -1;
+        if (cls >= 0) {
+            const int gt_before = wcnt[warp][2 * e] + __popc(same & gtm & lt);
+            const int eq_before = wcnt[warp][2 * e + 1] + __popc(same & eqm & lt);
+            if (cls == 0 || eq_before < st.need) r = st.base + gt_before + min(eq_before, st.need);
+        }
+        row_local[(size_t)s * K + k] = r;
+    }
 }
 
 __global__ void plan_finalize_kernel(const int32_t* __restrict__ idx, const int32_t* __restrict__ counts,
@@ -698,10 +723,22 @@
     return ab_round_up(kept + (int64_t)E * (row_align - 1), row_align);
 }
 
-extern "C" size_t ab_moe_plan_workspace_bytes(int S, int K, int E) {
-    (void)E;
-    return (size_t)ab_round_up((int64_t)S * K * sizeof(int32_t), 256);
-}
+namespace {
+struct PlanWs { size_t hist_off, zero_bytes, sel_off, cc_off, total; };
+PlanWs plan_ws(int S, int K, int E) {
+    PlanWs p;
+    size_t o = ab_round_up((int64_t)S * K * sizeof(int32_t), 256);
+    p.hist_off = o;
+    p.zero_bytes = ab_round_up(((int64_t)4 * E * K * 256 + 16) * sizeof(int), 256);
+    o += p.zero_bytes;
+    p.sel_off = o; o += ab_round_up((int64_t)E * K * sizeof(PlanSel), 256);
+    p.cc_off = o; o += ab_round_up(ab_ceil_div(S, PLAN_CHUNK) * K * 2 * E * (int64_t)sizeof(int), 256);
+    p.total = o;
+    return p;
+}
+}
+
+extern "C" size_t ab_moe_plan_workspace_bytes(int S, int K, int E) { return plan_ws(S, K, E).total; }
 
 extern "C" int ab_moe_plan(const int32_t* idx, const float* w, const int32_t* active, int cap, int32_t* counts,
                            int32_t* seg_off, int32_t* row_of, int32_t* tok_of_row, int32_t* slot_of_row,
@@ -715,15 +752,27 @@
         AB_REQUIRE(row_align > 0 && max_rows % row_align == 0 && max_rows >= ab_moe_max_rows(S, K, E, cap < S ? cap : S, row_align),
                    "moe_plan: max_rows %lld too small or not a multiple of %d", (long long)max_rows, row_align);
     }
-    AB_REQUIRE(ws && ws_bytes >= ab_moe_plan_workspace_bytes(S, K, E), "moe_plan: workspace too small");
+    const PlanWs pw = plan_ws(S, K, E);
+    AB_REQUIRE(ws && ws_bytes >= pw.total, "moe_plan: workspace too small");
+    unsigned char* w8 = (unsigned char*)ws;
     int32_t* row_local = (int32_t*)ws;
+    int* ghist = (int*)(w8 + pw.hist_off);
+    int* tickets = ghist + (size_t)4 * E * K * 256;
+    int* any_select = tickets + 8;
+    PlanSel* sel = (PlanSel*)(w8 + pw.sel_off);
+    int* cc = (int*)(w8 + pw.cc_off);
+    AB_CHECK_CUDA(cudaMemsetAsync(ghist, 0, pw.zero_bytes, stream));
     AB_CHECK_CUDA(cudaMemsetAsync(tok_of_row, 0xFF, (size_t)max_rows * sizeof(int32_t), stream));
     AB_CHECK_CUDA(cudaMemsetAsync(slot_of_row, 0xFF, (size_t)max_rows * sizeof(int32_t), stream));
-    int list_cap = (200 * 1024) / 8;
-    if (list_cap > S) list_cap = S;
-    const size_t plan_smem = (size_t)list_cap * sizeof(uint2);
-    AB_CHECK_CUDA(cudaFuncSetAttribute(plan_count_kernel, cudaFuncAttributeMaxDynamicSharedMemorySize, (int)plan_smem));
-    plan_count_kernel<<<E, PLAN_THREADS, plan_smem, stream>>>(idx, w, active, cap, counts, row_local, S, K, list_cap);
+    const dim3 hgrid((unsigned)ab_ceil_div(S, HIST_TOKENS), K), cgrid((unsigned)ab_ceil_div(S, PLAN_CHUNK), K);
+    for (int pass = 3; pass >= 0; --pass) {
+        plan_hist_kernel<<<hgrid, PLAN_THREADS, 0, stream>>>(idx, w, active, cap, pass, ghist + (size_t)(3 - pass) * E * K * 256, sel,
+                                                             any_select, tickets + (3 - pass), counts, S, K, E);
+        AB_LAUNCH_CHECK();
+    }
+    plan_chunk_count_kernel<<<cgrid, PLAN_THREADS, 0, stream>>>(idx, w, sel, cc, S, K, E);
+    AB_LAUNCH_CHECK();
+    plan_pos_kernel<<<cgrid, PLAN_THREADS, 0, stream>>>(idx, w, sel, cc, row_local, S, K, E);
     AB_LAUNCH_CHECK();
     const int64_t want = ab_ceil_div((int64_t)S * K, 256);
     const int grid = (int)(want < ab_num_sms() * 4 ? want : ab_num_sms() * 4);
diff --git a/apertis_llm_b200/csrc/moe_router.cu b/apertis_llm_b200/csrc/moe_router.cu
--- a/apertis_llm_b200/csrc/moe_router.cu
+++ b/apertis_llm_b200/csrc/moe_router.cu
@@ -16,6 +16,27 @@
 template <typename T>
 __device__ __forceinline__ void row_load(const T* row, int i, float* f) {
     ab_vec16<T>::unpack(__ldg(reinterpret_cast<const uint4*>(row) + i), f);
+}
+
+template <typename T>
+__device__ __forceinline__ void ld4g(const T* p, float* f) {
+    if constexpr (sizeof(T) == 4) {
+        const float4 q = __ldg(reinterpret_cast<const float4*>(p));
+        f[0] = q.x; f[1] = q.y; f[2] = q.z; f[3] = q.w;
+    } else {
+        const uint2 r = __ldg(reinterpret_cast<const uint2*>(p));
+        f[0] = __uint_as_float(r.x << 16); f[1] = __uint_as_float(r.x & 0xffff0000u);
+        f[2] = __uint_as_float(r.y << 16); f[3] = __uint_as_float(r.y & 0xffff0000u);
+    }
+}
+template <typename T>
+__device__ __forceinline__ void ab_st4(T* p, const float* o) {
+    if constexpr (sizeof(T) == 4) {
+        *reinterpret_cast<float4*>(p) = make_float4(o[0], o[1], o[2], o[3]);
+    } else {
+        __nv_bfloat162 lo = __floats2bfloat162_rn(o[0], o[1]), hi = __floats2bfloat162_rn(o[2], o[3]);
+        *reinterpret_cast<uint2*>(p) = make_uint2(*reinterpret_cast<uint32_t*>(&lo), *reinterpret_cast<uint32_t*>(&hi));
+    }
 }
 
 __device__ __forceinline__ void select_topk(float logit, int lane, int E, int K, float& g, float& lse, int& my_idx, float& my_p,
@@ -215,7 +236,16 @@
 }
 
 template <typename T, int EM, int NV>
-__global__ void __launch_bounds__(WARPS * 32, (NV * ab_vec16<T>::N <= 24 && EM <= 8) ? 4 : 1) router_fwd_reg_kernel(const T* __restrict__ x, const float* __restrict__ ln_w,
+#ifndef FWD_MINB
+#define FWD_MINB 2
+#endif
+#ifndef FWD_REGPF
+#define FWD_REGPF 1
+#endif
+#ifndef FWD_PERSIST
+#define FWD_PERSIST 1
+#endif
+__global__ void __launch_bounds__(WARPS * 32, (NV * ab_vec16<T>::N <= 24 && EM <= 8) ? FWD_MINB : 1) router_fwd_reg_kernel(const T* __restrict__ x, const float* __restrict__ ln_w,
                                                                     const float* __restrict__ ln_b, float eps,
                                                                     const float* __restrict__ Wr, const float* __restrict__ br,
                                                                     const float* __restrict__ noise,
@@ -250,20 +280,43 @@
     const int nvec = Dm / V;
     const float inv_dm = 1.0f / (float)Dm;
     float a_g = 0.f, a_cnt = 0.f, a_l2 = 0.f;
-    for (int s = blockIdx.x * WARPS + warp; s < S; s += gridDim.x * WARPS) {
+    constexpr bool PF = FWD_REGPF && NV * V <= 64;
+    float fn[NV][V];
+    auto load_row = [&](int s) {
         const T* row = x + (size_t)s * Dm;
-        float f[NV][V];
-        float sum = 0.f;
 #pragma unroll
         for (int i = 0; i < NV; ++i) {
             const int iv = i * 32 + lane;
-            if (iv < nvec) {
-                row_load<T>(row, iv, f[i]);
+            if (s < S && iv < nvec) {
+                row_load<T>(row, iv, fn[i]);
+            } else {
+#pragma unroll
+                for (int v = 0; v < V; ++v) fn[i][v] = 0.f;
+            }
+        }
+    };
+    const int stride = gridDim.x * WARPS;
+    if constexpr (PF) load_row(blockIdx.x * WARPS + warp);
+    for (int s = blockIdx.x * WARPS + warp; s < S; s += stride) {
+        if constexpr (!PF) {
+            load_row(s);
+            const char* nx = reinterpret_cast<const char*>(x + (size_t)(s + stride) * Dm);
+            if (s + stride < S)
+                for (int o = lane * 128; o < Dm * (int)sizeof(T); o += 32 * 128) asm volatile("prefetch.global.L2 [%0];" ::"l"(nx + o));
+        }
+        float f[NV][V];
+#pragma unroll
+        for (int i = 0; i < NV; ++i) {
+#pragma unroll
+            for (int v = 0; v < V; ++v) f[i][v] = fn[i][v];
+        }
+        if constexpr (PF) load_row(s + stride);
+        float sum = 0.f;
+#pragma unroll
+        for (int i = 0; i < NV; ++i) {
+            if (i * 32 + lane < nvec) {
 #pragma unroll
                 for (int v = 0; v < V; ++v) sum += f[i][v];
-            } else {
-#pragma unroll
-                for (int v = 0; v < V; ++v) f[i][v] = 0.f;
             }
         }
         const float mean = ab_warp_sum(sum) * inv_dm;
@@ -363,6 +416,63 @@
         select_topk(l, lane, E, K, g, lse, my_idx, my_p, den, sel_mask);
         write_selection(s, lane, E, K, g, lse, my_idx, my_p, den, gates, idx, probs, w, lse_out);
     }
+}
+
+__device__ __forceinline__ void router_token_grad(int s, int lane, int E, int K, int Dm, const float* GS, const float* cvec,
+                                                  const float* __restrict__ stats, const float* __restrict__ gates,
+                                                  const int32_t* __restrict__ idx, const float* __restrict__ probs,
+                                                  const float* __restrict__ lse, const float* __restrict__ lclean,
+                                                  const float* __restrict__ noise, const float* __restrict__ f, float g_lb,
+                                                  float g_rz, const float* __restrict__ dw_row, const int32_t* __restrict__ row_of,
+                                                  int& my_r, float& dl, float& mean, float& rstd, float& m1, float& m2,
+                                                  float& a_db, float& a_dn) {
+    const float g_in = lane < E ? gates[(size_t)s * E + lane] : 0.f;
+    const float lse_s = lse[s];
+    const float lc_in = lane < E ? lclean[(size_t)s * E + lane] : 0.f;
+    const float nz_in = noise != nullptr && lane < E ? noise[(size_t)s * E + lane] : 0.f;
+    const float f_in = lane < E ? f[lane] : 0.f;
+    mean = stats[2 * (size_t)s]; rstd = stats[2 * (size_t)s + 1];
+    int my_i = 0;
+    float my_dw = 0.f, my_pk = 0.f;
+    my_r = -1;
+    if (lane < K) {
+        my_r = row_of[(size_t)s * K + lane];
+        my_i = idx[(size_t)s * K + lane];
+        my_pk = probs[(size_t)s * K + lane];
+        my_dw = my_r >= 0 ? dw_row[my_r] : 0.f;
+    }
+    float den = 0.f;
+    for (int k = 0; k < K; ++k) den += __shfl_sync(0xffffffffu, my_pk, k);
+    den += 1e-6f;
+    const float dot = ab_warp_sum(my_dw * my_pk);
+    const float inv = 1.f / den;
+    const float my_dp = my_dw * inv - dot * inv * inv;
+    float dgate = 0.f, g = 0.f;
+    for (int k = 0; k < K; ++k) {
+        const int ik = __shfl_sync(0xffffffffu, my_i, k);
+        const float dpk = __shfl_sync(0xffffffffu, my_dp, k);
+        if (lane == ik) dgate += dpk;
+    }
+    if (lane < E) {
+        g = g_in;
+        dgate = fmaf(g_lb, f_in, dgate);
+    } else {
+        dgate = 0.f;
+    }
+    const float gd = ab_warp_sum(g * dgate);
+    dl = 0.f;
+    if (lane < E) {
+        dl = g * (dgate - gd) + g_rz * 2.f * lse_s * g;
+        a_db += dl;
+        if (noise) a_dn = fmaf(dl, nz_in, a_dn);
+    }
+    float t1 = 0.f, t2 = 0.f;
+    if (lane < E) {
+        t1 = dl * GS[lane];
+        t2 = dl * (lc_in - cvec[lane]);
+    }
+    m1 = ab_warp_sum(t1) / (float)Dm;
+    m2 = ab_warp_sum(t2) / (float)Dm;
 }
 
 template <typename T, int EM>
@@ -401,48 +511,11 @@
     const int nvec = Dm / V;
     float a_db = 0.f, a_dn = 0.f;
     for (int s = blockIdx.x * WARPS + warp; s < S; s += gridDim.x * WARPS) {
-        int my_r = -1, my_i = 0;
-        float my_dw = 0.f, my_pk = 0.f;
-        if (lane < K) {
-            my_r = row_of[(size_t)s * K + lane];
-            my_i = idx[(size_t)s * K + lane];
-            my_pk = probs[(size_t)s * K + lane];
-            my_dw = my_r >= 0 ? dw_row[my_r] : 0.f;
-        }
-        float den = 0.f;
-        for (int k = 0; k < K; ++k) den += __shfl_sync(0xffffffffu, my_pk, k);
-        den += 1e-6f;
-        const float dot = ab_warp_sum(my_dw * my_pk);
-        const float inv = 1.f / den;
-        const float my_dp = my_dw * inv - dot * inv * inv;
-        float dgate = 0.f, g = 0.f;
-        for (int k = 0; k < K; ++k) {
-            const int ik = __shfl_sync(0xffffffffu, my_i, k);
-            const float dpk = __shfl_sync(0xffffffffu, my_dp, k);
-            if (lane == ik) dgate += dpk;
-        }
-        if (lane < E) {
-            g = gates[(size_t)s * E + lane];
-            dgate = fmaf(g_lb, f[lane], dgate);
-        } else {
-            dgate = 0.f;
-        }
-        const float gd = ab_warp_sum(g * dgate);
-        float dl = 0.f;
-        if (lane < E) {
-            dl = g * (dgate - gd) + g_rz * 2.f * lse[s] * g;
-            dlogits[(size_t)s * E + lane] = dl;
-            a_db += dl;
-            if (noise) a_dn = fmaf(dl, noise[(size_t)s * E + lane], a_dn);
-        }
-        const float mean = stats[2 * (size_t)s], rstd = stats[2 * (size_t)s + 1];
-        float t1 = 0.f, t2 = 0.f;
-        if (lane < E) {
-            t1 = dl * GS[lane];
-            t2 = dl * (lclean[(size_t)s * E + lane] - cvec[lane]);
-        }
-        const float m1 = ab_warp_sum(t1) / (float)Dm;
-        const float m2 = ab_warp_sum(t2) / (float)Dm;
+        int my_r;
+        float dl, mean, rstd, m1, m2;
+        router_token_grad(s, lane, E, K, Dm, GS, cvec, stats, gates, idx, probs, lse, lclean, noise, f, g_lb, g_rz, dw_row, row_of,
+                          my_r, dl, mean, rstd, m1, m2, a_db, a_dn);
+        if (lane < E) dlogits[(size_t)s * E + lane] = dl;
         float dle[EM];
 #pragma unroll
         for (int e = 0; e < EM; ++e) dle[e] = __shfl_sync(0xffffffffu, dl, e);
@@ -542,6 +615,189 @@
         if (e < E) qpart[((size_t)blockIdx.y * E + e) * Dm + d] = acc[e];
 }
 
+constexpr int TSC = 12;
+constexpr int TOK_CTAS_PER_SM = 6;
+constexpr int FUSED_EM = 8;
+__global__ void __launch_bounds__(WARPS * 32, TOK_CTAS_PER_SM) router_bwd_tok_kernel(const float* __restrict__ stats, const float* __restrict__ ln_w,
+                                                                    const float* __restrict__ ln_b, const float* __restrict__ Wr,
+                                                                    const float* __restrict__ br, const float* __restrict__ gates,
+                                                                    const int32_t* __restrict__ idx, const float* __restrict__ probs,
+                                                                    const float* __restrict__ lse, const float* __restrict__ lclean,
+                                                                    const float* __restrict__ noise, const float* __restrict__ f,
+                                                                    const float* __restrict__ scal, const float* __restrict__ dw_row,
+                                                                    const int32_t* __restrict__ row_of, float* __restrict__ tsc,
+                                                                    float* __restrict__ part, int S, int Dm, int E, int K) {
+    __shared__ float GS[32], cvec[32], red[WARPS][2 * FUSED_EM];
+    const int tid = threadIdx.x, lane = tid & 31, warp = tid >> 5;
+    for (int e = warp; e < E; e += WARPS) {
+        float a1 = 0.f, a2 = 0.f;
+        for (int d = lane; d < Dm; d += 32) {
+            a1 = fmaf(ln_w[d], Wr[(size_t)e * Dm + d], a1);
+            a2 = fmaf(ln_b[d], Wr[(size_t)e * Dm + d], a2);
+        }
+        a1 = ab_warp_sum(a1); a2 = ab_warp_sum(a2);
+        if (lane == 0) { GS[e] = a1; cvec[e] = a2 + br[e]; }
+    }
+    __syncthreads();
+    const float g_lb = scal[0], g_rz = scal[1];
+    float a_db = 0.f, a_dn = 0.f;
+    for (int s = blockIdx.x * WARPS + warp; s < S; s += gridDim.x * WARPS) {
+        int my_r;
+        float dl, mean, rstd, m1, m2;
+        router_token_grad(s, lane, E, K, Dm, GS, cvec, stats, gates, idx, probs, lse, lclean, noise, f, g_lb, g_rz, dw_row, row_of,
+                          my_r, dl, mean, rstd, m1, m2, a_db, a_dn);
+        float v = dl;
+        if (lane == 8) v = mean;
+        if (lane == 9) v = rstd;
+        if (lane == 10) v = m1;
+        if (lane == 11) v = m2;
+        if (lane < TSC) tsc[(size_t)s * TSC + lane] = v;
+    }
+    const int NA = 2 * E;
+    if (lane < E) { red[warp][lane] = a_db; red[warp][E + lane] = a_dn; }
+    __syncthreads();
+    if (tid < NA) {
+        float s2 = 0.f;
+        for (int wv = 0; wv < WARPS; ++wv) s2 += red[wv][tid];
+        part[(size_t)blockIdx.x * NA + tid] = s2;
+    }
+}
+
+constexpr int BT = 32;
+constexpr int FUSED_MAX_THREADS = 256;
+constexpr int FUSED_MAX_REGS = 144;
+template <typename T, int KM>
+__global__ void __maxnreg__(FUSED_MAX_REGS) router_bwd_col_kernel(const T* __restrict__ x, const float* __restrict__ ln_w,
+                                                                  const float* __restrict__ Wr, const float* __restrict__ tsc,
+                                                                  const float* __restrict__ dxrow, const int32_t* __restrict__ row_of,
+                                                                  T* __restrict__ dx, float* __restrict__ qpart, int S, int Dm,
+                                                                  int E, int K) {
+    constexpr int EM = FUSED_EM;
+    constexpr int U = KM <= 2 ? 4 : 1;
+    constexpr int NSC = BT * TSC, NROW = BT * KM;
+    extern __shared__ float sm[];
+    float* Wsm = sm;
+    float* stile = Wsm + (size_t)E * Dm;
+    int* srow = reinterpret_cast<int*>(stile + 2 * NSC);
+    const int tid = threadIdx.x;
+    for (int i = tid; i < E * Dm; i += blockDim.x) Wsm[i] = Wr[i];
+    const int d = 4 * tid;
+    const bool has_col = d < Dm;
+    float gg[4] = {0.f, 0.f, 0.f, 0.f};
+    if (has_col) {
+        const float4 gq = __ldg(reinterpret_cast<const float4*>(ln_w + d));
+        gg[0] = gq.x; gg[1] = gq.y; gg[2] = gq.z; gg[3] = gq.w;
+    }
+    auto fetch = [&](int s0, int buf) {
+        const int nt = s0 < S ? min(BT, S - s0) : 0;
+        for (int i = tid; i < nt * TSC; i += blockDim.x) {
+            const unsigned dst = (unsigned)__cvta_generic_to_shared(stile + buf * NSC + i);
+            asm volatile("cp.async.ca.shared.global [%0], [%1], 4;" ::"r"(dst), "l"(tsc + (size_t)s0 * TSC + i));
+        }
+        for (int i = tid; i < nt * KM; i += blockDim.x) {
+            const int j = i / KM, k = i % KM;
+            if (k < K) {
+                const unsigned dst = (unsigned)__cvta_generic_to_shared(srow + buf * NROW + i);
+                asm volatile("cp.async.ca.shared.global [%0], [%1], 4;" ::"r"(dst), "l"(row_of + (size_t)(s0 + j) * K + k));
+            } else {
+                srow[buf * NROW + i] = -1;
+            }
+        }
+    };
+    float q[EM][4];
+#pragma unroll
+    for (int e = 0; e < EM; ++e) { q[e][0] = q[e][1] = q[e][2] = q[e][3] = 0.f; }
+    const int step = gridDim.x * BT;
+    fetch(blockIdx.x * BT, 0);
+    asm volatile("cp.async.wait_all;" ::: "memory");
+    __syncthreads();
+    int buf = 0;
+    for (int s0 = blockIdx.x * BT; s0 < S; s0 += step, buf ^= 1) {
+        const int nt = min(BT, S - s0);
+        fetch(s0 + step, buf ^ 1);
+        const float* sc = stile + buf * NSC;
+        const int* rw = srow + buf * NROW;
+        if (has_col) {
+            for (int j0 = 0; j0 < nt; j0 += U) {
+#pragma unroll
+                for (int u = 0; u < U; ++u) {
+                    const int j = j0 + U + u;
+                    if (j < nt && (tid & 7) == 0) {
+                        asm volatile("prefetch.global.L2 [%0];" ::"l"(x + (size_t)(s0 + j) * Dm + d));
+#pragma unroll
+                        for (int k = 0; k < KM; ++k) {
+                            const int r = rw[j * KM + k];
+                            if (r >= 0) asm volatile("prefetch.global.L2 [%0];" ::"l"(dxrow + (size_t)r * Dm + d));
+                        }
+                    }
+                }
+                float xv[U][4], er[U][KM][4];
+#pragma unroll
+                for (int u = 0; u < U; ++u) {
+                    const int j = j0 + u;
+#pragma unroll
+                    for (int k = 0; k < KM; ++k) er[u][k][0] = er[u][k][1] = er[u][k][2] = er[u][k][3] = 0.f;
+                    xv[u][0] = xv[u][1] = xv[u][2] = xv[u][3] = 0.f;
+                    if (j < nt) {
+                        ld4g<T>(x + (size_t)(s0 + j) * Dm + d, xv[u]);
+#pragma unroll
+                        for (int k = 0; k < KM; ++k) {
+                            const int r = rw[j * KM + k];
+                            if (r >= 0) ld4g<float>(dxrow + (size_t)r * Dm + d, er[u][k]);
+                        }
+                    }
+                }
+#pragma unroll
+                for (int u = 0; u < U; ++u) {
+                    const int j = j0 + u;
+                    if (j >= nt) break;
+                    const float* t = sc + j * TSC;
+                    const float mean = t[8], rstd = t[9], m1 = t[10], m2 = t[11];
+                    float dle[EM];
+#pragma unroll
+                    for (int e = 0; e < EM; ++e) dle[e] = t[e];
+                    float dxn[4] = {0.f, 0.f, 0.f, 0.f};
+#pragma unroll
+                    for (int e = 0; e < EM; ++e) {
+                        if (e < E) {
+                            const float4 wq = *reinterpret_cast<const float4*>(Wsm + (size_t)e * Dm + d);
+                            dxn[0] = fmaf(dle[e], wq.x, dxn[0]); dxn[1] = fmaf(dle[e], wq.y, dxn[1]);
+                            dxn[2] = fmaf(dle[e], wq.z, dxn[2]); dxn[3] = fmaf(dle[e], wq.w, dxn[3]);
+                        }
+                    }
+                    float o[4], xh[4];
+#pragma unroll
+                    for (int v = 0; v < 4; ++v) {
+                        xh[v] = (xv[u][v] - mean) * rstd;
+                        o[v] = rstd * (dxn[v] * gg[v] - m1 - xh[v] * m2);
+                    }
+#pragma unroll
+                    for (int k = 0; k < KM; ++k) {
+                        if (rw[j * KM + k] >= 0) {
+#pragma unroll
+                            for (int v = 0; v < 4; ++v) o[v] += er[u][k][v];
+                        }
+                    }
+                    ab_st4<T>(dx + (size_t)(s0 + j) * Dm + d, o);
+#pragma unroll
+                    for (int e = 0; e < EM; ++e) {
+#pragma unroll
+                        for (int v = 0; v < 4; ++v) q[e][v] = fmaf(dle[e], xh[v], q[e][v]);
+                    }
+                }
+            }
+        }
+        asm volatile("cp.async.wait_all;" ::: "memory");
+        __syncthreads();
+    }
+    if (has_col) {
+#pragma unroll
+        for (int e = 0; e < EM; ++e)
+            if (e < E) *reinterpret_cast<float4*>(qpart + ((size_t)blockIdx.x * E + e) * Dm + d) = make_float4(q[e][0], q[e][1], q[e][2], q[e][3]);
+    }
+}
+
+int param_groups(int E) { const int g = 1024 / (32 * E); return g < 1 ? 1 : (g > 4 ? 4 : g); }
 __global__ void router_param_kernel(const float* __restrict__ qpart, int nqb, const float* __restrict__ part, int nparts,
                                     const float* __restrict__ ln_w, const float* __restrict__ ln_b, const float* __restrict__ Wr,
                                     float* __restrict__ dWr, float* __restrict__ dbr, float* __restrict__ dln_w,
@@ -549,23 +805,24 @@
     __shared__ float sdb[64];
     __shared__ float sgw[32][33], sgb[32][33];
     __shared__ float spart[16][64];
-    const int tx = threadIdx.x, e = threadIdx.y;
-    const int tid = e * 32 + tx;
-    const int nthr = 32 * E;
+    __shared__ float sq[32][33];
+    const int tx = threadIdx.x, e = threadIdx.y, grp = threadIdx.z, G = blockDim.z;
+    const int tid = (grp * E + e) * 32 + tx;
+    const int nthr = 32 * E * G;
     {
         const int ncol = 2 * E;
         const int ngrp = min(16, nthr / ncol);
-        const int col = tid % ncol, grp = tid / ncol;
-        if (grp < ngrp) {
+        const int col = tid % ncol, pg = tid / ncol;
+        if (pg < ngrp) {
             float s = 0.f;
-            for (int r0 = grp; r0 < nparts; r0 += ngrp * 4) {
+            for (int r0 = pg; r0 < nparts; r0 += ngrp * 4) {
                 float v[4];
 #pragma unroll
                 for (int u = 0; u < 4; ++u) v[u] = r0 + u * ngrp < nparts ? part[(size_t)(r0 + u * ngrp) * ncol + col] : 0.f;
 #pragma unroll
                 for (int u = 0; u < 4; ++u) s += v[u];
             }
-            spart[grp][col] = s;
+            spart[pg][col] = s;
         }
         __syncthreads();
         if (tid < ncol) {
@@ -578,27 +835,36 @@
             }
         }
     }
-    __syncthreads();
     const int d = blockIdx.x * 32 + tx;
-    float gw = 0.f, gb = 0.f;
-    if (d < Dm) {
+    {
         float q = 0.f;
-        for (int r0 = 0; r0 < nqb; r0 += 8) {
-            float qv[8];
-#pragma unroll
-            for (int u = 0; u < 8; ++u) qv[u] = r0 + u < nqb ? qpart[((size_t)(r0 + u) * E + e) * Dm + d] : 0.f;
-#pragma unroll
-            for (int u = 0; u < 8; ++u) q += qv[u];
-        }
-        const float wv = Wr[(size_t)e * Dm + d];
-        dWr[(size_t)e * Dm + d] = fmaf(ln_w[d], q, ln_b[d] * sdb[e]);
-        gw = wv * q;
-        gb = wv * sdb[e];
-    }
-    sgw[e][tx] = gw;
-    sgb[e][tx] = gb;
-    __syncthreads();
-    if (e == 0 && d < Dm) {
+        if (d < Dm) {
+            for (int r0 = grp; r0 < nqb; r0 += 8 * G) {
+                float qv[8];
+#pragma unroll
+                for (int u = 0; u < 8; ++u) qv[u] = r0 + u * G < nqb ? qpart[((size_t)(r0 + u * G) * E + e) * Dm + d] : 0.f;
+#pragma unroll
+                for (int u = 0; u < 8; ++u) q += qv[u];
+            }
+        }
+        sq[grp * E + e][tx] = q;
+    }
+    __syncthreads();
+    if (grp == 0) {
+        float gw = 0.f, gb = 0.f;
+        if (d < Dm) {
+            float q = 0.f;
+            for (int g2 = 0; g2 < G; ++g2) q += sq[g2 * E + e][tx];
+            const float wv = Wr[(size_t)e * Dm + d];
+            dWr[(size_t)e * Dm + d] = fmaf(ln_w[d], q, ln_b[d] * sdb[e]);
+            gw = wv * q;
+            gb = wv * sdb[e];
+        }
+        sgw[e][tx] = gw;
+        sgb[e][tx] = gb;
+    }
+    __syncthreads();
+    if (grp == 0 && e == 0 && d < Dm) {
         float a = 0.f, b = 0.f;
         for (int i = 0; i < E; ++i) { a += sgw[i][tx]; b += sgb[i][tx]; }
         dln_w[d] = a;
@@ -620,14 +886,21 @@
     w.total = ab_round_up((int64_t)w.grid * (2 * E + 1) * sizeof(float), 256);
     return w;
 }
-struct BwdWs { size_t part_off, dl_off, q_off, total; int grid, nqb; };
+constexpr int MAX_FUSED_PER_SM = 4;
+int tok_grid(int S) {
+    const int want = (int)ab_ceil_div(S, WARPS);
+    const int cap = ab_num_sms() * TOK_CTAS_PER_SM;
+    return want < cap ? want : cap;
+}
+bool bwd_fused(int Dm, int E) { return E <= FUSED_EM && Dm % 4 == 0 && Dm / 4 <= FUSED_MAX_THREADS; }
+struct BwdWs { size_t part_off, dl_off, q_off, total; int nqb; };
 BwdWs bwd_ws(int S, int Dm, int E) {
     BwdWs w;
-    w.grid = router_grid(S);
-    w.nqb = (int)ab_ceil_div(S, qb_for(em_for(E)));
+    const bool fused = bwd_fused(Dm, E);
+    w.nqb = fused ? ab_num_sms() * MAX_FUSED_PER_SM : (int)ab_ceil_div(S, qb_for(em_for(E)));
     size_t o = 0;
-    w.part_off = o; o += ab_round_up((int64_t)w.grid * 2 * E * sizeof(float), 256);
-    w.dl_off = o; o += ab_round_up((int64_t)S * E * sizeof(float), 256);
+    w.part_off = o; o += ab_round_up((int64_t)(fused ? tok_grid(S) : router_grid(S)) * 2 * E * sizeof(float), 256);
+    w.dl_off = o; o += ab_round_up((int64_t)S * (fused ? TSC : E) * sizeof(float), 256);
     w.q_off = o; o += ab_round_up((int64_t)w.nqb * E * Dm * sizeof(float), 256);
     w.total = o;
     return w;
@@ -660,12 +933,17 @@
     float* part = (float*)ws;
     const int V = dtype == AB_F32 ? 4 : 8;
     const int nv = (int)ab_ceil_div(Dm, 32 * V);
+    int grid = wl.grid;
 #define AB_ROUTER_LAUNCH(KERNEL)                                                                                        \
     {                                                                                                                    \
         auto k = KERNEL;                                                                                                 \
         AB_CHECK_CUDA(cudaFuncSetAttribute(k, cudaFuncAttributeMaxDynamicSharedMemorySize, (int)smem));                 \
-        k<<<wl.grid, WARPS * 32, smem, stream>>>((const TT*)x, ln_w, ln_b, eps, Wr, br, noise, noise_scale, lclean,     \
-                                                 logits, gates, idx, probs, w, lse, stats_out, part, S, Dm, E, K, quant); \
+        int occ = 4;                                                                                                     \
+        if (FWD_PERSIST) AB_CHECK_CUDA(cudaOccupancyMaxActiveBlocksPerMultiprocessor(&occ, k, WARPS * 32, smem));       \
+        occ = occ < 1 ? 1 : (occ > 4 ? 4 : occ);                                                                        \
+        grid = wl.grid < ab_num_sms() * occ ? wl.grid : ab_num_sms() * occ;                                              \
+        k<<<grid, WARPS * 32, smem, stream>>>((const TT*)x, ln_w, ln_b, eps, Wr, br, noise, noise_scale, lclean,         \
+                                              logits, gates, idx, probs, w, lse, stats_out, part, S, Dm, E, K, quant);    \
     }
 #define AB_ROUTER_FWD(TT_, EMV)                                                                                         \
     {                                                                                                                    \
@@ -684,7 +962,7 @@
 #undef AB_ROUTER_LAUNCH
 #undef AB_ROUTER_FWD
     AB_LAUNCH_CHECK();
-    reduce_rows_kernel<<<(unsigned)ab_ceil_div(2 * E + 1, 4), 128, 0, stream>>>(part, wl.grid, 2 * E + 1, aux);
+    reduce_rows_kernel<<<(unsigned)ab_ceil_div(2 * E + 1, 4), 128, 0, stream>>>(part, grid, 2 * E + 1, aux);
     AB_LAUNCH_CHECK();
     return AB_OK;
 }
@@ -713,27 +991,56 @@
     float* part = (float*)(w8 + wl.part_off);
     float* dl = (float*)(w8 + wl.dl_off);
     float* qpart = (float*)(w8 + wl.q_off);
-    const size_t smem = ((size_t)E * Dm + Dm + 64 + WARPS * 2 * E) * sizeof(float);
-    dim3 qgrid((unsigned)ab_ceil_div(Dm, 256), wl.nqb);
+    int nqb = wl.nqb, nparts = router_grid(S);
+    if (bwd_fused(Dm, E)) {
+        nparts = tok_grid(S);
+        router_bwd_tok_kernel<<<nparts, WARPS * 32, 0, stream>>>(stats, ln_w, ln_b, Wr, br, gates, idx, probs, lse, lclean, noise, f,
+                                                                 scal, dw_row, row_of, dl, part, S, Dm, E, K);
+        AB_LAUNCH_CHECK();
+        const int threads = (int)ab_round_up(Dm / 4 > 64 ? Dm / 4 : 64, 32);
+        const size_t smem = ((size_t)E * Dm + 2 * BT * TSC + 2 * BT * MAX_K) * sizeof(float);
+#define AB_ROUTER_BWD_COL(TT, KMV)                                                                                      \
+    {                                                                                                                    \
+        auto k = router_bwd_col_kernel<TT, KMV>;                                                                         \
+        AB_CHECK_CUDA(cudaFuncSetAttribute(k, cudaFuncAttributeMaxDynamicSharedMemorySize, (int)smem));                 \
+        int occ = 0;                                                                                                     \
+        AB_CHECK_CUDA(cudaOccupancyMaxActiveBlocksPerMultiprocessor(&occ, k, threads, smem));                           \
+        occ = occ < 1 ? 1 : (occ > MAX_FUSED_PER_SM ? MAX_FUSED_PER_SM : occ);                                          \
+        const int64_t want = ab_ceil_div(S, BT);                                                                         \
+        nqb = (int)(want < (int64_t)ab_num_sms() * occ ? want : (int64_t)ab_num_sms() * occ);                            \
+        k<<<nqb, threads, smem, stream>>>((const TT*)x, ln_w, Wr, dl, dxrow, row_of, (TT*)dx, qpart, S, Dm, E, K);        \
+    }
+        if (dtype == AB_F32) {
+            if (K <= 2) AB_ROUTER_BWD_COL(float, 2) else AB_ROUTER_BWD_COL(float, MAX_K)
+        } else {
+            if (K <= 2) AB_ROUTER_BWD_COL(__nv_bfloat16, 2) else AB_ROUTER_BWD_COL(__nv_bfloat16, MAX_K)
+        }
+#undef AB_ROUTER_BWD_COL
+        AB_LAUNCH_CHECK();
+    } else {
+        const size_t smem = ((size_t)E * Dm + Dm + 64 + WARPS * 2 * E) * sizeof(float);
+        dim3 qgrid((unsigned)ab_ceil_div(Dm, 256), nqb);
 #define AB_ROUTER_BWD(TT, EMV)                                                                                          \
     {                                                                                                                    \
         auto k = router_bwd_kernel<TT, EMV>;                                                                             \
         AB_CHECK_CUDA(cudaFuncSetAttribute(k, cudaFuncAttributeMaxDynamicSharedMemorySize, (int)smem));                 \
-        k<<<wl.grid, WARPS * 32, smem, stream>>>((const TT*)x, stats, ln_w, ln_b, Wr, br, gates, idx, probs, lse,       \
-                                                 lclean, noise, f, scal, dw_row, dxrow, row_of, (TT*)dx, dl, part, S,   \
-                                                 Dm, E, K);                                                              \
+        k<<<nparts, WARPS * 32, smem, stream>>>((const TT*)x, stats, ln_w, ln_b, Wr, br, gates, idx, probs, lse,        \
+                                                lclean, noise, f, scal, dw_row, dxrow, row_of, (TT*)dx, dl, part, S,    \
+                                                Dm, E, K);                                                               \
         AB_LAUNCH_CHECK();                                                                                               \
         router_q_kernel<TT, EMV><<<qgrid, 256, 0, stream>>>((const TT*)x, stats, dl, qpart, S, Dm, E);                  \
     }
-    if (dtype == AB_F32) {
-        if (E <= 8) AB_ROUTER_BWD(float, 8) else if (E <= 16) AB_ROUTER_BWD(float, 16) else AB_ROUTER_BWD(float, 32)
-    } else {
-        if (E <= 8) AB_ROUTER_BWD(__nv_bfloat16, 8) else if (E <= 16) AB_ROUTER_BWD(__nv_bfloat16, 16) else AB_ROUTER_BWD(__nv_bfloat16, 32)
-    }
+        if (dtype == AB_F32) {
+            if (E <= 8) AB_ROUTER_BWD(float, 8) else if (E <= 16) AB_ROUTER_BWD(float, 16) else AB_ROUTER_BWD(float, 32)
+        } else {
+            if (E <= 8) AB_ROUTER_BWD(__nv_bfloat16, 8) else if (E <= 16) AB_ROUTER_BWD(__nv_bfloat16, 16) else AB_ROUTER_BWD(__nv_bfloat16, 32)
+        }
 #undef AB_ROUTER_BWD
-    AB_LAUNCH_CHECK();
-    router_param_kernel<<<(unsigned)ab_ceil_div(Dm, 32), dim3(32, E), 0, stream>>>(qpart, wl.nqb, part, wl.grid, ln_w, ln_b, Wr, dWr,
-                                                                                  dbr, dln_w, dln_b, dnoise_scale, Dm, E);
+        AB_LAUNCH_CHECK();
+    }
+    const int G = param_groups(E);
+    router_param_kernel<<<(unsigned)ab_ceil_div(Dm, 32), dim3(32, E, G), 0, stream>>>(qpart, nqb, part, nparts, ln_w, ln_b, Wr, dWr,
+                                                                                     dbr, dln_w, dln_b, dnoise_scale, Dm, E);
     AB_LAUNCH_CHECK();
     return AB_OK;
 }
```
